# silverlight6/Ultrasound_Modeling

Measured on AMD Instinct MI355X. Metric: segmentation training images/sec at 256x256, higher is better.
Workload: dtype bf16

## Files before the change

### include/usseg.h

```cpp
#ifndef USSEG_H
#define USSEG_H

#include <stddef.h>
#include <stdint.h>

#ifdef __cplusplus
extern "C" {
#endif

typedef void* usseg_stream_t;

typedef enum UssegStatus {
  USSEG_OK = 0,
  USSEG_ERR_BAD_ARG = -1,
  USSEG_ERR_UNSUPPORTED = -2,
  USSEG_ERR_LAUNCH = -3
} UssegStatus;

typedef enum UssegAct { USSEG_ACT_NONE = 0, USSEG_ACT_LRELU = 1, USSEG_ACT_RELU = 2, USSEG_ACT_ELU = 3, USSEG_ACT_GELU = 4 } UssegAct;

enum {
  USSEG_OUT_F32 = 1,
  USSEG_ACCUMULATE = 2
};

typedef struct UssegConvDesc {
  int32_t B, H, W;
  int32_t Cin, Cout;
  int32_t ldx, ldy;
  int32_t ksize;
  int32_t dilation;
  int32_t act;
  float alpha;
  int32_t flags;
} UssegConvDesc;

const char* usseg_last_error(void);
int usseg_version(void);

int usseg_conv2d_fwd(const UssegConvDesc* d, const void* x, const void* wp_fwd, const float* bias,
                     const void* residual, int32_t ldr, void* y, usseg_stream_t stream);
int usseg_conv2d_fwd_affine(const UssegConvDesc* d, const void* x, const void* wp_fwd, const float* scale, const float* shift,
                            const void* residual, int32_t ldr, void* y, usseg_stream_t stream);
typedef struct UssegBnFoldJob {
  const float *gamma, *beta, *mean, *var;
  const float* bias;
  float *scale, *shift;
  int32_t C, Cp;
  float eps;
  int32_t reserved;
} UssegBnFoldJob;
int usseg_bn_fold_batched(const UssegBnFoldJob* jobs_dev, int32_t njobs, usseg_stream_t stream);
int usseg_conv2d_dgrad(const UssegConvDesc* d, const void* dy, const void* wp_dgrad, const void* residual,
                       int32_t ldr, void* dx, usseg_stream_t stream);
int usseg_conv2d_wgrad(const UssegConvDesc* d, const void* x, const void* dy, float* dw_scratch, float* ws,
                       int64_t ws_floats, usseg_stream_t stream);

int usseg_conv2d_dgrad_branches(const UssegConvDesc* d, int32_t nbranches, const int32_t* ksize, const int32_t* dilation,
                                const int32_t* ch_off, int32_t Cb, const void* dy, const void* wp_cat, const void* residual,
                                int32_t ldr, void* dx, usseg_stream_t stream);

typedef struct UssegWgradBlock {
  float* dst;
  int64_t sT, sI, sO;
  int32_t i_off, o_off, ni, no;
} UssegWgradBlock;
typedef struct UssegWgradDst {
  int32_t nblocks;
  int32_t reserved;
  UssegWgradBlock blk[4];
} UssegWgradDst;
int usseg_conv2d_wgrad_mapped(const UssegConvDesc* d, const void* x, const void* dy, const UssegWgradDst* dst, float* ws,
                              int64_t ws_floats, usseg_stream_t stream);
int usseg_tconv2d_wgrad_mapped(const UssegConvDesc* d, const void* x, const void* dy, const UssegWgradDst* dst, float* ws,
                               int64_t ws_floats, usseg_stream_t stream);

typedef struct UssegWgradJob {
  UssegConvDesc desc;
  const void* x;
  const void* dy;
  float* dw;
  const UssegWgradDst* dst;
} UssegWgradJob;
int usseg_conv2d_wgrad_multi(int32_t njobs, const UssegWgradJob* jobs, float* ws, int64_t ws_floats, usseg_stream_t stream);

int usseg_defer_begin(usseg_stream_t stream, float* reduce_ws, int64_t reduce_floats, float* wgrad_ws, int64_t wgrad_floats);
int usseg_defer_flush(usseg_stream_t stream);
int usseg_defer_end(usseg_stream_t stream);

typedef struct UssegConvJob {
  UssegConvDesc desc;
  const void* x;
  const void* wp;
  const float* bias;
  const void* residual;
  int32_t ldr;
  int32_t reserved;
  void* y;
  const float* scale;
} UssegConvJob;
int usseg_conv2d_fwd_multi(int32_t njobs, const UssegConvJob* jobs, usseg_stream_t stream);
int usseg_conv2d_dgrad_multi(int32_t njobs, const UssegConvJob* jobs, usseg_stream_t stream);

int usseg_tconv2d_fwd(const UssegConvDesc* d, const void* x, const void* wp_fwd, const float* bias, void* y,
                      usseg_stream_t stream);
int usseg_tconv2d_dgrad(const UssegConvDesc* d, const void* dy, const void* wp_dgrad, const void* residual,
                        int32_t ldr, void* dx, usseg_stream_t stream);
int usseg_tconv2d_wgrad(const UssegConvDesc* d, const void* x, const void* dy, float* dw_scratch,
                        usseg_stream_t stream);

int usseg_pack_weight(const float* src, int64_t sT, int64_t sN, int64_t sK, int32_t T, int32_t Nn, int32_t Kk,
                      void* dst, int32_t Kw, int32_t tap_stride, int32_t n_off, int32_t k_off,
                      usseg_stream_t stream);
typedef struct UssegPackJob {
  const float* src;
  void* dst;
  int64_t sT, sN, sK;
  int32_t T, Nn, Kk, Kw, tap_stride, n_off, k_off, reserved;
  const float* nscale;
} UssegPackJob;
int usseg_pack_weights_batched(const UssegPackJob* jobs_dev, int32_t njobs, usseg_stream_t stream);
int usseg_pack_weights_flat(const UssegPackJob* jobs_dev, const int32_t* tilemap_dev, int32_t nblocks, usseg_stream_t stream);
int usseg_unpack_wgrad(const float* scratch, int32_t Mrows, int32_t Ncols, int32_t T, int32_t Nn, int32_t Kk,
                       int32_t n_off, int32_t k_off, float* dst, int64_t sT, int64_t sN, int64_t sK,
                       float scale, int32_t accumulate, usseg_stream_t stream);
typedef struct UssegUnpackJob {
  const float* scratch;
  float* dst;
  int64_t sT, sN, sK;
  int32_t Mrows, Ncols, T, Nn, Kk, n_off, k_off, accumulate;
  float scale;
  int32_t reserved;
} UssegUnpackJob;
int usseg_unpack_wgrad_batched(const UssegUnpackJob* jobs_dev, int32_t njobs, int32_t max_elems, usseg_stream_t stream);

typedef struct UssegNormDesc {
  int64_t M;
  int32_t C, Cphys;
  int32_t ldx, ldy;
  int32_t G;
  int32_t mode;
  float eps;
  int32_t act;
  float alpha;
  int32_t lddx;
} UssegNormDesc;
int usseg_norm_act_fwd(const UssegNormDesc* d, const void* x, const float* gamma, const float* beta,
                       const float* mean, const float* var, const void* mask, int32_t ldm, void* y, usseg_stream_t stream);
int usseg_dropout_mask(void* mask, int64_t M, int32_t C, int32_t ld, uint64_t seed, float rate, usseg_stream_t stream);
int usseg_dropout_mask_step(void* mask, int64_t M, int32_t C, int32_t ld, uint64_t seed, const int32_t* step_dev, float rate,
                            usseg_stream_t stream);
int usseg_counter_add(int32_t* counter, int32_t inc, usseg_stream_t stream);
int usseg_norm_act_bwd(const UssegNormDesc* d, const void* x, const void* dy, const float* gamma, const float* beta,
                       const float* mean, const float* var, const void* mask, int32_t ldm, void* dx, float* dgamma,
                       float* dbeta, float* dbias, float* ws, usseg_stream_t stream);
int usseg_norm_act_bwd_res(const UssegNormDesc* d, const void* x, const void* dy, const float* gamma, const float* beta,
                           const void* dres, int32_t lddres, void* dx, float* dgamma, float* dbeta, float* dbias, float* ws,
                           usseg_stream_t stream);
int usseg_norm_act_fwd_gap(const UssegNormDesc* d, const void* x, const float* gamma, const float* beta, const float* mean,
                           const float* var, void* y, int32_t B, int32_t nb, float* gap_rows, usseg_stream_t stream);
int usseg_norm_act_bwd_sa(const UssegNormDesc* d, const void* x, const void* dout, const float* gamma, const float* beta,
                          const float* mean, const float* var, int32_t B, const float* sa_s, const float* sa_dg, float sa_mult,
                          void* dx, float* dgamma, float* dbeta, float* dbias, float* ws, usseg_stream_t stream);
int usseg_norm_act_bwd_pair(const UssegNormDesc* da, const void* xa, const void* dya, const float* gamma_a, const float* beta_a, void* dxa,
                            float* dgamma_a, float* dbeta_a, float* dbias_a, const UssegNormDesc* db, const void* xb, const void* doutb,
                            const float* gamma_b, const float* beta_b, int32_t B, const float* sa_s, const float* sa_dg, float sa_mult, void* dxb,
                            float* dgamma_b, float* dbeta_b, float* dbias_b, float* ws, usseg_stream_t stream);
int usseg_stem_fwd(int32_t B, int32_t H, int32_t W, const void* x, int32_t ldx, const void* w1, const float* b1, const void* w2, const float* b2,
                   const void* w3, const float* b3, const float* gamma, const float* beta, const float* mean, const float* var, float eps,
                   float alpha, void* y1, void* t1, void* c2, void* pooled, usseg_stream_t stream);
int usseg_stem_fwd_infer(int32_t B, int32_t H, int32_t W, const void* x, int32_t ldx, const void* w1, const float* b1, const void* w2,
                         const float* b2, const void* w3, const float* b3, const float* gamma, const float* beta, const float* mean,
                         const float* var, float eps, float alpha, void* pooled, usseg_stream_t stream);
int usseg_conv3_dgrad_actbwd(int32_t B, int32_t H, int32_t W, const void* dy, int32_t lddy, const void* wd, int32_t Co, const void* yact, int32_t ldy,
                             int32_t mode, const float* gamma, const float* beta, const float* var, float eps, float alpha, void* dx,
                             int32_t lddx, float* dgamma, float* dbeta, float* dbias, float* ws, usseg_stream_t stream);
typedef struct UssegCardinalDesc {
  int32_t B, H, W;
  int32_t Cin;
  int32_t P, cv11, cvkk;
  int32_t Up, Vp, Oc;
  int32_t ldx, ldu, ldv, ldsc;
  float eps, alpha;
} UssegCardinalDesc;
int32_t usseg_cardinal_supported(const UssegCardinalDesc* d);
int usseg_cardinal_fwd(const UssegCardinalDesc* d, const void* x, const void* w1, const float* b1, const float* g1, const float* be1,
                       const void* w2, const float* b2, const float* g2, const float* be2, const void* wsc, const float* bsc,
                       const float* gsc, const float* besc, void* u_raw, void* u, void* v_raw, void* y, float* gap_rows, void* sc_raw,
                       void* sc, usseg_stream_t stream);
int usseg_cardinal_fwd_infer(const UssegCardinalDesc* d, const void* x, const void* w1, const float* b1, const float* g1, const float* be1,
                             const void* w2, const float* b2, const float* g2, const float* be2, const void* wsc, const float* bsc,
                             const float* gsc, const float* besc, void* y, float* gap_rows, void* sc, usseg_stream_t stream);
int usseg_cardinal_bwd(const UssegCardinalDesc* d, const void* dout, int32_t ldo, const void* dsc, int32_t lddsc, const void* v_raw,
                       const void* u_raw, const void* sc_raw, const void* w2d, const float* g2, const float* be2, const float* g1,
                       const float* be1, const float* gsc, const float* besc, const float* sa_s, const float* sa_dg, float sa_mult, void* dv,
                       void* dcat, int32_t ldc, float* dg2, float* dbe2, float* db2, float* dg1, float* dbe1, float* db1, float* dgsc,
                       float* dbesc, float* dbsc, float* ws, usseg_stream_t stream);
int usseg_bn_act_pool_fwd(const void* x, int32_t B, int32_t H, int32_t W, int32_t C, int32_t Cphys, int32_t ldx, const float* gamma,
                          const float* beta, const float* mean, const float* var, float eps, int32_t act, float alpha, void* y,
                          int32_t ldy, usseg_stream_t stream);
int usseg_bn_act_pool_bwd(const void* x, const void* dy, int32_t B, int32_t H, int32_t W, int32_t C, int32_t Cphys, int32_t ldx,
                          int32_t lddy, const float* gamma, const float* beta, const float* mean, const float* var, float eps,
                          int32_t act, float alpha, void* dx, int32_t lddx, float* dgamma, float* dbeta, float* dbias, float* ws,
                          usseg_stream_t stream);
int64_t usseg_reduce_ws_floats(void);
int usseg_channel_stats(const void* x, int64_t M, int32_t C, int32_t ldx, float* sum, float* sumsq, float* ws,
                        usseg_stream_t stream);

int usseg_bn_finalize_stats(const float* sum, const float* sumsq, int64_t M, int32_t C, float momentum, float* mean, float* var,
                            float* moving_mean, float* moving_var, usseg_stream_t stream);
int usseg_bn_batch_stats(const void* x, int64_t M, int32_t C, int32_t ldx, float momentum, float* mean, float* var, float* moving_mean,
                         float* moving_var, float* ws, usseg_stream_t stream);
int usseg_bn_train_bwd_fix(const void* x, void* dx, int64_t M, int32_t C, int32_t Cphys, int32_t ldx, int32_t lddx, const float* gamma,
                           const float* mean, const float* var, float eps, const float* tg, const float* tb, usseg_stream_t stream);

int usseg_act_fwd(const void* x, int64_t M, int32_t C, int32_t ldx, int32_t ldy, int32_t act, float alpha, void* y,
                  usseg_stream_t stream);
int usseg_act_bwd(const void* x, const void* dy, int64_t M, int32_t C, int32_t ldx, int32_t lddy, int32_t lddx,
                  int32_t act, float alpha, void* dx, usseg_stream_t stream);
int usseg_act_bwd_colsum(const void* x, const void* dy, int64_t M, int32_t C, int32_t ldx, int32_t lddy, int32_t lddx, int32_t act,
                         float alpha, void* dx, float* db, float* ws, usseg_stream_t stream);

int usseg_avgpool2_fwd(const void* x, int32_t B, int32_t H, int32_t W, int32_t C, int32_t ldx, int32_t ldy, void* y,
                       usseg_stream_t stream);
int usseg_avgpool2_bwd(const void* dy, int32_t B, int32_t H, int32_t W, int32_t C, int32_t lddy, int32_t lddx,
                       const void* add, int32_t ldadd, void* dx, usseg_stream_t stream);
int usseg_avgpool2_bwd_colsum(const void* dy, int32_t B, int32_t H, int32_t W, int32_t C, int32_t lddy, int32_t lddx, const void* add,
                              int32_t ldadd, void* dx, float* db, float* ws, usseg_stream_t stream);

int usseg_copy_channels(const void* src, int64_t M, int32_t C, int32_t lds, void* dst, int32_t ldd, int32_t accumulate,
                        usseg_stream_t stream);
int usseg_cast_input(const void* src, int32_t src_is_f64, int64_t M, int32_t C, void* dst, int32_t Cphys,
                     usseg_stream_t stream);
int usseg_cast_bf16_to_f32(const void* src, int64_t M, int32_t C, int32_t lds, float* dst, usseg_stream_t stream);

typedef struct UssegSplitAttnDesc {
  int32_t B, HW;
  int32_t P, R, Cg, Hd;
  int32_t ldy, ldo;
  int32_t Cy_phys, Co_phys;
  float mult;
  int32_t norm_mode;
  float eps;
  int32_t act;
  float alpha;
  int32_t use_sigmoid;
} UssegSplitAttnDesc;
typedef struct UssegSplitAttnParams {
  const float *w1, *b1, *gamma, *beta, *mean, *var, *w2, *b2;
} UssegSplitAttnParams;
typedef struct UssegSplitAttnGrads {
  float *w1, *b1, *gamma, *beta, *w2, *b2;
} UssegSplitAttnGrads;
int usseg_splitattn_gap(const UssegSplitAttnDesc* d, const void* y, float* g, float* ws, usseg_stream_t stream);
int64_t usseg_splitattn_ws_floats(const UssegSplitAttnDesc* d);
int usseg_splitattn_mlp_fwd(const UssegSplitAttnDesc* d, const float* g, int32_t g_rows, int32_t g_stride,
                            const UssegSplitAttnParams* p, float* s, float* ws, usseg_stream_t stream);
int usseg_splitattn_apply_fwd(const UssegSplitAttnDesc* d, const void* y, const float* s, void* out,
                              usseg_stream_t stream);
int usseg_splitattn_apply_bwd_reduce(const UssegSplitAttnDesc* d, const void* y, const void* dout, int32_t lddo,
                                     float* ds, float* ws, usseg_stream_t stream);
int64_t usseg_splitattn_mlp_bwd_ws_floats(const UssegSplitAttnDesc* d);
int usseg_splitattn_mlp_bwd(const UssegSplitAttnDesc* d, const float* g, int32_t g_rows, int32_t g_stride,
                            const UssegSplitAttnParams* p, const float* s, const float* ws, const float* ds, float* dg,
                            const UssegSplitAttnGrads* grads, float* grad_ws, usseg_stream_t stream);
int usseg_splitattn_bwd_fused(const UssegSplitAttnDesc* d, const void* y, const void* dout, int32_t lddo, const float* g, int32_t g_rows,
                              int32_t g_stride, const UssegSplitAttnParams* p, const float* s, const float* ws, float* dg,
                              const UssegSplitAttnGrads* grads, float* reduce_ws, float* grad_ws, usseg_stream_t stream);
int usseg_splitattn_apply_bwd_dy(const UssegSplitAttnDesc* d, const void* dout, int32_t lddo, const float* s,
                                 const float* dg, void* dy, int32_t lddy, usseg_stream_t stream);

typedef struct UssegLossDesc {
  int64_t M;
  int32_t HW;
  int32_t C, ldl, lddl;
  int32_t loss_kind;
  float label_smoothing;
  float clip_eps;
  float inv_global_batch;
  int32_t quad_w;
} UssegLossDesc;
#define USSEG_ACC_FLOATS 2050
int usseg_softmax_loss_fwd_bwd(const UssegLossDesc* d, const float* logits, const float* y_true, const float* scale,
                               float* probs, float* loss, void* dlogits, usseg_stream_t stream);
int usseg_head_quad_softmax_loss(const void* x, int32_t B, int32_t h, int32_t w, int32_t Cin_phys, int32_t ldx, const void* wq, const float* bias, int32_t C,
                                 const float* y_true, float* probs, float* loss, void* dlogits, float label_smoothing, float clip_eps,
                                 float inv_global_batch, usseg_stream_t stream);
int usseg_accuracy(const float* probs, const float* y_true, int64_t M, int32_t C, float* acc, usseg_stream_t stream);
typedef struct UssegSegCountDesc {
  int32_t B, H, W, C;
  int32_t num_classes;
  int32_t round;
} UssegSegCountDesc;
#define USSEG_SEG_COUNTS 23
int usseg_seg_counts(const UssegSegCountDesc* d, const float* y_true, const float* y_pred, uint64_t* counts, usseg_stream_t stream);
int usseg_cascade_gate(const float* probs, int32_t C_mask, int64_t M, const void* x, int32_t ldx, void* x_gated, uint8_t* mask,
                       usseg_stream_t stream);
int usseg_cascade_maps(const float* probs, int32_t C, int64_t M, float* prob_map, float* bleed_prob, usseg_stream_t stream);
int usseg_loss_from_probs(const UssegLossDesc* d, const float* probs, const float* y_true, const float* scale, float* loss,
                          usseg_stream_t stream);
typedef struct UssegClassLoss {
  float w[8];
  float gamma;
  float factor;
} UssegClassLoss;
int usseg_softmax_loss_fwd_bwd_cl(const UssegLossDesc* d, const UssegClassLoss* cl, const float* logits, const float* y_true, float* probs,
                                  float* loss, void* dlogits, usseg_stream_t stream);
int usseg_head_quad_softmax_loss_cl(const void* x, int32_t B, int32_t h, int32_t w, int32_t Cin_phys, int32_t ldx, const void* wq, const float* bias,
                                    int32_t C, const float* y_true, float* probs, float* loss, void* dlogits, float label_smoothing, float clip_eps,
                                    float inv_global_batch, const UssegClassLoss* cl, usseg_stream_t stream);
int usseg_loss_from_probs_cl(const UssegLossDesc* d, const UssegClassLoss* cl, const float* probs, const float* y_true, float* loss,
                             int32_t as_map, usseg_stream_t stream);
typedef struct UssegOverlapLoss {
  float w[8];
  float alpha;
  float beta;
  float smooth;
  float power;
  float ov_weight;
  float ce_weight;
} UssegOverlapLoss;
#define USSEG_OVERLAP_ACC_FLOATS 8224
int usseg_overlap_loss_grid(int64_t M);
int usseg_overlap_loss_sums(const UssegLossDesc* d, const UssegOverlapLoss* ol, float ov_scale, const float* probs, const float* y_true,
                            float* acc, int64_t acc_floats, usseg_stream_t stream);
int usseg_overlap_loss_bwd(const UssegLossDesc* d, const UssegOverlapLoss* ol, const float* probs, const float* y_true, const float* acc,
                           int64_t acc_floats, void* dlogits, usseg_stream_t stream);
int64_t usseg_sdf_ws_bytes(int32_t B, int32_t H, int32_t W, int32_t C);
int usseg_sdf_labels(const float* y_true, int32_t B, int32_t H, int32_t W, int32_t C, float thr, float* phi, void* ws, int64_t ws_bytes,
                     usseg_stream_t stream);
int64_t usseg_surface_ws_bytes(int32_t N, int32_t H, int32_t W);
int usseg_surface_dist(const uint8_t* a, const uint8_t* b, int32_t N, int32_t H, int32_t W, int64_t* counters, double* sums, void* ws,
                       int64_t ws_bytes, usseg_stream_t stream);
int64_t usseg_surface_stats_ws_bytes(int32_t N, int32_t H, int32_t W);
int usseg_surface_stats(const uint8_t* a, const uint8_t* b, int32_t N, int32_t H, int32_t W, const double* quant, int32_t P, const int32_t* tol2,
                        int32_t T, int64_t* counters, double* sums, int32_t* sel, int64_t* within, void* ws, int64_t ws_bytes,
                        usseg_stream_t stream);
int64_t usseg_components_ws_bytes(int32_t N, int32_t H, int32_t W);
int usseg_label_components(const uint8_t* mask, int32_t N, int32_t H, int32_t W, int32_t connectivity, int32_t* labels, int32_t* count, void* ws,
                           int64_t ws_bytes, usseg_stream_t stream);
int usseg_component_stats(const int32_t* labels, const float* prob, int32_t N, int32_t H, int32_t W, int32_t cap, int64_t* stats,
                          usseg_stream_t stream);
int usseg_clean_mask(const uint8_t* mask, const float* prob, int32_t N, int32_t H, int32_t W, int32_t connectivity, int32_t min_area,
                     float min_peak, uint8_t* out, void* ws, int64_t ws_bytes, usseg_stream_t stream);
int usseg_component_overlap(const int32_t* labels_a, const int32_t* labels_b, int32_t N, int32_t H, int32_t W, int32_t cap_a, int32_t cap_b,
                            int32_t* hit_a, int32_t* hit_b, usseg_stream_t stream);
typedef struct UssegBoundaryLoss {
  float u[8];
} UssegBoundaryLoss;
int usseg_overlap_boundary_loss_sums(const UssegLossDesc* d, const UssegOverlapLoss* ol, float ov_scale, const float* probs, const float* y_true,
                                     const float* phi, const UssegBoundaryLoss* bl, const float* wb, float* acc, int64_t acc_floats,
                                     usseg_stream_t stream);
int usseg_overlap_boundary_loss_bwd(const UssegLossDesc* d, const UssegOverlapLoss* ol, const float* probs, const float* y_true, const float* phi,
                                    const UssegBoundaryLoss* bl, const float* acc, int64_t acc_floats, void* dlogits, usseg_stream_t stream);
#define USSEG_SORT_TILE 2048
#define USSEG_SORT_DIGIT_BITS 8
int64_t usseg_sort_ws_bytes(int32_t S, int64_t n);
int usseg_sort_pairs_u32(const uint32_t* keys_in, const uint32_t* vals_in, int32_t S, int64_t n, int32_t key_bits, uint32_t* keys_out,
                         uint32_t* vals_out, void* ws, int64_t ws_bytes, usseg_stream_t stream);
typedef struct UssegLovaszLoss {
  float w[8];
  float lv_weight;
  float ce_weight;
  float threshold;
  int32_t all_classes;
} UssegLovaszLoss;
int64_t usseg_lovasz_ws_bytes(int64_t M, int32_t C);
int usseg_lovasz_coeffs(const UssegLossDesc* d, UssegLovaszLoss ll, const float* probs, const float* y_true, float* g, int32_t* counts, void* ws,
                        int64_t ws_bytes, usseg_stream_t stream);
int usseg_lovasz_loss_sums(const UssegLossDesc* d, UssegLovaszLoss ll, float ov_scale, const float* probs, const float* y_true, const float* g,
                           const int32_t* counts, float* acc, int64_t acc_floats, usseg_stream_t stream);
int usseg_lovasz_loss_bwd(const UssegLossDesc* d, UssegLovaszLoss ll, const float* probs, const float* y_true, const float* g, const float* acc,
                          int64_t acc_floats, void* dlogits, usseg_stream_t stream);
int usseg_quad_bias_expand(const float* bias, int32_t C, int32_t Np, float* out , usseg_stream_t stream);
int usseg_quad_bias_fold(const float* d16 , int32_t C, float* dbias, usseg_stream_t stream);
int usseg_tconv_quad_unpack(const float* dq, int32_t Cin_phys, int32_t Cin, int32_t Cout, int32_t Np, int32_t ksize, float* grad,
                            usseg_stream_t stream);
int usseg_quad_head_fold(const float* dq, int32_t Cin_phys, int32_t Cin, int32_t Cout, int32_t Np, int32_t ksize, float* grad, const float* d16,
                         float* dbias, usseg_stream_t stream);
int usseg_space_to_depth2(const void* full, int32_t B, int32_t H, int32_t W, int32_t C, int32_t ld_full, void* quad, int32_t Np,
                          int32_t ld_quad, int32_t to_quad, usseg_stream_t stream);
int usseg_tconv_quad_fwd(const UssegConvDesc* d, int32_t ksize, int32_t Np, const void* x, const void* wq_f, const float* bias_q, void* y4,
                         usseg_stream_t stream);
int usseg_tconv_quad_dgrad(const UssegConvDesc* d, int32_t ksize, int32_t Np, const void* dy4, const void* wq_d, void* dx, usseg_stream_t stream);
int usseg_tconv_quad_wgrad(const UssegConvDesc* d, int32_t ksize, int32_t Np, const void* x, const void* dy4, float* dq, float* ws,
                           int64_t ws_floats, usseg_stream_t stream);

int usseg_loss_cat_scale(const float* y_true, int32_t B, int32_t HW, int32_t C, float* scale, usseg_stream_t stream);

int usseg_label2vec(const float* label, int64_t M, int32_t num_classes, float* out, usseg_stream_t stream);
typedef struct UssegAugSample {
  int32_t do_reduc, nclip;
  int32_t clip[2][4];
  int32_t do_shift, shift_r, shift_c, shift_dir;
  int32_t do_noise, do_flip;
  uint64_t seed;
} UssegAugSample;
typedef struct UssegAugDesc {
  int32_t B, H, W, C;
  int32_t Cphys;
  int32_t num_classes;
} UssegAugDesc;
int usseg_augment(const UssegAugDesc* d, const UssegAugSample* samples_dev, const void* x, int32_t x_is_f64, const float* y,
                  const float* noise, void* x_out_bf16, float* x_out_f32, float* y_out, float* y_vec, usseg_stream_t stream);

int usseg_reinject_hidden(void* hidden, int64_t numel, int32_t n, void* const* bufs, const int32_t* c0, const int32_t* ld,
                          int32_t backward, usseg_stream_t stream);

int usseg_patchify(const void* x, int32_t x_is_f64, int32_t B, int32_t H, int32_t W, int32_t C, int32_t patch, void* out, int32_t Cp,
                   usseg_stream_t stream);
int usseg_patch_merge(void* full, int32_t B, int32_t H, int32_t W, int32_t C, int32_t ldf, void* merged, int32_t ldm, int32_t backward,
                      usseg_stream_t stream);
int usseg_ln_wide_fwd(const void* x, int64_t M, int32_t C, int32_t ldx, const float* gamma, const float* beta, float eps, void* y,
                      int32_t ldy, usseg_stream_t stream);
int usseg_ln_wide_bwd(const void* x, const void* dy, int64_t M, int32_t C, int32_t ldx, int32_t lddy, const float* gamma, float eps,
                      void* dx, int32_t lddx, float* dgamma, float* dbeta, float* ws, int64_t ws_floats, usseg_stream_t stream);
int usseg_window_attn_fwd(const void* qkv, int32_t ldq, const float* table, int32_t B, int32_t H, int32_t W, int32_t C, int32_t heads,
                          int32_t ws, int32_t shift, void* out, int32_t ldo, usseg_stream_t stream);
int64_t usseg_window_attn_bwd_ws_floats(int32_t B, int32_t H, int32_t W, int32_t heads, int32_t ws);
int usseg_window_attn_bwd(const void* qkv, int32_t ldq, const void* dout, int32_t ldo, const float* table, int32_t B, int32_t H, int32_t W,
                          int32_t C, int32_t heads, int32_t ws, int32_t shift, void* dqkv, float* dtable, float* ws_rows,
                          usseg_stream_t stream);
int usseg_token_mean_fwd(const void* x, int32_t B, int32_t L, int32_t C, int32_t ld, float* out, usseg_stream_t stream);
int usseg_token_mean_bwd(const float* dy, int32_t B, int32_t L, int32_t C, int32_t ld, void* dx, usseg_stream_t stream);

int usseg_colsum(const void* dy, int64_t M, int32_t C, int32_t ld, float* db, float* ws, usseg_stream_t stream);

int usseg_sumsq(const float* g, int64_t n, float* out, usseg_stream_t stream);
int usseg_sum_f32(const float* x, int64_t n, float* out, usseg_stream_t stream);
int usseg_sumsq_advance(const float* g, int64_t n, float* out, int32_t* step, float* lr_t_dev, float lr, float beta1, float beta2,
                        usseg_stream_t stream);
int usseg_adam_clip_step(float* p, const float* g, float* m, float* v, int64_t n, const float* sumsq, float clip_norm,
                         const float* lr_t_dev, float beta1, float beta2, float eps, usseg_stream_t stream);
int usseg_adam_advance(int32_t* step, float* lr_t_dev, float lr, float beta1, float beta2, usseg_stream_t stream);
int usseg_fill_f32(float* p, int64_t n, float value, usseg_stream_t stream);
int usseg_scale_f32(float* p, int64_t n, const float* sumsq, float clip_norm, usseg_stream_t stream);

#define USSEG_SCHED_MAX_PIECES 16
typedef struct UssegLrSchedule {
  int32_t n;
  int32_t boundary[USSEG_SCHED_MAX_PIECES - 1];
  float lr[USSEG_SCHED_MAX_PIECES];
  float wd[USSEG_SCHED_MAX_PIECES];
} UssegLrSchedule;
int usseg_sched_advance(int32_t* step, const UssegLrSchedule* sched_dev, float* lr_t_dev, float* wd_t_dev, float beta1, float beta2,
                        usseg_stream_t stream);
int usseg_sumsq_sched_advance(const float* g, int64_t n, float* out, int32_t* step, const UssegLrSchedule* sched_dev, float* lr_t_dev,
                              float* wd_t_dev, float beta1, float beta2, usseg_stream_t stream);
int usseg_adamw_step(float* p, const float* g, float* m, float* v, int64_t n, const float* sumsq, float clip_norm, const float* lr_t_dev,
                     const float* wd_t_dev, const uint8_t* decay_mask, float beta1, float beta2, float eps, usseg_stream_t stream);

typedef struct UssegGemmDesc {
  int32_t M, N, K;
  int32_t ldx, ldw, ldy;
  int32_t nb1, nb2;
  int64_t xs1, xs2, ws1, ws2, ys1, ys2;
  int32_t flags;
} UssegGemmDesc;
int usseg_gemm_nt_batched(const UssegGemmDesc* d, const void* x, const void* w, void* y, usseg_stream_t stream);
int usseg_gemm_tn_batched(const UssegGemmDesc* d, const void* a, const void* b, float* out, usseg_stream_t stream);
int usseg_softmax_rows_fwd(const float* s, int64_t rows, int32_t n, float scale, float* p32, void* pbf, usseg_stream_t stream);
int usseg_softmax_rows_bwd(const float* p32, const float* dp, int64_t rows, int32_t n, float scale, void* ds_bf, usseg_stream_t stream);
int usseg_transpose_batched(const void* src, int32_t R, int32_t C, int32_t lds, int32_t nb1, int32_t nb2, int64_t ss1, int64_t ss2,
                            void* dst, usseg_stream_t stream);
int usseg_cast_f32_to_bf16_batched(const float* src, int32_t R, int32_t C, int32_t nb1, int32_t nb2, void* dst, int32_t ldd, int64_t ds1,
                                   int64_t ds2, usseg_stream_t stream);

typedef struct UssegFlashDesc {
  int32_t B, N, H, head_dim;
  int32_t ld_qkv, ld_o;
  float scale;
} UssegFlashDesc;
int usseg_flash_attn_fwd(const UssegFlashDesc* d, const void* q, const void* k, const void* v, void* o, float* o32, float* lse,
                         usseg_stream_t stream);
int usseg_flash_attn_bwd(const UssegFlashDesc* d, const void* q, const void* k, const void* v, const void* o, const float* o32,
                         const void* d_o, const float* lse, float* delta, void* dq, void* dk, void* dv, usseg_stream_t stream);

int usseg_prof_enable(int32_t kind_mask, int32_t capacity);
int usseg_prof_read(int32_t kind, double* total_ms, int64_t* launches);
int usseg_prof_disable(void);

#define USSEG_PREP_H 256
#define USSEG_PREP_W 80
int usseg_prep_cycle_stats(const double* frames, int32_t C, int32_t H0, int32_t W0, double* col_ws, double* stats, usseg_stream_t stream);
int usseg_prep_label(const double* brain, int32_t Hb, int32_t Wb, const double* blood, const double* normal, int32_t Hm, int32_t Wm,
                     int32_t objective, float* ws, float* label, uint8_t* gate, usseg_stream_t stream);
int usseg_prep_label_thick(const double* brain, int32_t Hb, int32_t Wb, const double* blood, int32_t Hm, int32_t Wm, int32_t order,
                           float* label, uint8_t* gate, usseg_stream_t stream);
int usseg_prep_assemble(const double* frames, const double* stats, int32_t C, int32_t H0, int32_t W0, const double* bmode, int32_t Hq,
                        int32_t Wq, int32_t F, const float* label, const uint8_t* gate, int32_t objective, double* out, usseg_stream_t stream);

int usseg_select_ranks_f64(const double* x, int32_t N, int64_t n, const int32_t* ranks, int32_t R, const int32_t* active, double* out,
                           usseg_stream_t stream);
#define USSEG_PREP_AUG_PARTIALS 64
typedef struct UssegPrepAugSample {
  int32_t do_flip, do_reduc, do_contrast, do_clip;
  int32_t clip[4];
  int32_t do_rotate, rot_slot;
  int32_t do_shift, shift_r, shift_c, shift_dir;
  int32_t do_noise, reserved;
  uint64_t seed;
  double rot[6];
} UssegPrepAugSample;
typedef struct UssegPrepAugDesc {
  int32_t N, H, W, C;
  int32_t n_rot;
  int32_t k_lo, k_hi;
  double g_lo, g_hi;
  double zH, zW;
} UssegPrepAugDesc;
int64_t usseg_prep_aug_ws_doubles(int32_t N, int32_t H, int32_t W, int32_t C, int32_t n_rot);
int usseg_prep_aug(const UssegPrepAugDesc* d, const UssegPrepAugSample* samples_dev, const int32_t* rot_list_dev, const double* x,
                   const double* noise, double* ws, int64_t ws_doubles, double* out, double* noise_out, usseg_stream_t stream);

int usseg_cone_index(const double* X, const double* Y, int32_t H, int32_t W, double xmin, double ymin, double ppu, int32_t Hp, int32_t Wp,
                     int32_t* index, usseg_stream_t stream);
int usseg_cone_range(const double* bmode, int32_t B, int32_t HW, double* range, int32_t* nonfinite, usseg_stream_t stream);
int usseg_cone_render(const int32_t* index, int32_t Hp, int32_t Wp, int32_t gap, const float* prob_map, const double* label, const float* bleed,
                      const double* bmode, int32_t B, int32_t H, int32_t W, const double* ranges, const double* bmode_range, const uint8_t* luts,
                      uint8_t* out, usseg_stream_t stream);

#define USSEG_ENSEMBLE_MAX 16
#define USSEG_CALIB_MAX_BINS 64
typedef struct UssegEnsembleDesc {
  int32_t B, H, W, C;
  int32_t K;
} UssegEnsembleDesc;
int usseg_ensemble_merge(const UssegEnsembleDesc* d, const float* const* members, uint32_t flip_w, float* mean_probs, float* entropy,
                         float* mutual_info, float* variance, usseg_stream_t stream);
int usseg_ensemble_image_scores(const UssegEnsembleDesc* d, const float* mean_probs, const float* entropy, const float* mutual_info,
                                float* scores, int32_t* counts, usseg_stream_t stream);
typedef struct UssegCalibDesc {
  int32_t B, H, W, C;
  int32_t bins;
  int32_t cls;
} UssegCalibDesc;
int usseg_calibration_bins(const UssegCalibDesc* d, const float* probs, const float* y_true, int64_t* counts, usseg_stream_t stream);

#ifdef __cplusplus
}
#endif
#endif
```

### ultrasound_modeling_amd/_lib.py

```python
from __future__ import annotations

import ctypes as C
import os

import torch
from . import knobs

_HERE = os.path.dirname(os.path.abspath(__file__))
LIB_PATH = knobs.get("USSEG_LIB") or os.path.join(_HERE, "libusseg_hip.so")

c_i32, c_i64, c_f32, c_vp = C.c_int32, C.c_int64, C.c_float, C.c_void_p


class UssegError(RuntimeError):
    pass


class ConvDesc(C.Structure):
    _fields_ = [("B", c_i32), ("H", c_i32), ("W", c_i32), ("Cin", c_i32), ("Cout", c_i32), ("ldx", c_i32),
                ("ldy", c_i32), ("ksize", c_i32), ("dilation", c_i32), ("act", c_i32), ("alpha", c_f32),
                ("flags", c_i32)]


class ConvJob(C.Structure):
    _fields_ = [("desc", ConvDesc), ("x", c_vp), ("wp", c_vp), ("bias", c_vp), ("residual", c_vp), ("ldr", c_i32),
                ("reserved", c_i32), ("y", c_vp), ("scale", c_vp)]


class WgradBlock(C.Structure):
    _fields_ = [("dst", c_vp), ("sT", c_i64), ("sI", c_i64), ("sO", c_i64), ("i_off", c_i32), ("o_off", c_i32), ("ni", c_i32), ("no", c_i32)]


class WgradDst(C.Structure):
    _fields_ = [("nblocks", c_i32), ("reserved", c_i32), ("blk", WgradBlock * 4)]


P_WgradDst = C.POINTER(WgradDst)


class WgradJob(C.Structure):
    _fields_ = [("desc", ConvDesc), ("x", c_vp), ("dy", c_vp), ("dw", c_vp), ("dst", P_WgradDst)]


class AugSample(C.Structure):
    _fields_ = [("do_reduc", c_i32), ("nclip", c_i32), ("clip", (c_i32 * 4) * 2), ("do_shift", c_i32), ("shift_r", c_i32),
                ("shift_c", c_i32), ("shift_dir", c_i32), ("do_noise", c_i32), ("do_flip", c_i32), ("seed", C.c_uint64)]


class AugDesc(C.Structure):
    _fields_ = [("B", c_i32), ("H", c_i32), ("W", c_i32), ("C", c_i32), ("Cphys", c_i32), ("num_classes", c_i32)]


class PrepAugSample(C.Structure):
    _fields_ = [("do_flip", c_i32), ("do_reduc", c_i32), ("do_contrast", c_i32), ("do_clip", c_i32), ("clip", c_i32 * 4), ("do_rotate", c_i32),
                ("rot_slot", c_i32), ("do_shift", c_i32), ("shift_r", c_i32), ("shift_c", c_i32), ("shift_dir", c_i32), ("do_noise", c_i32),
                ("reserved", c_i32), ("seed", C.c_uint64), ("rot", C.c_double * 6)]


class PrepAugDesc(C.Structure):
    _fields_ = [("N", c_i32), ("H", c_i32), ("W", c_i32), ("C", c_i32), ("n_rot", c_i32), ("k_lo", c_i32), ("k_hi", c_i32),
                ("g_lo", C.c_double), ("g_hi", C.c_double), ("zH", C.c_double), ("zW", C.c_double)]


class NormDesc(C.Structure):
    _fields_ = [("M", c_i64), ("C", c_i32), ("Cphys", c_i32), ("ldx", c_i32), ("ldy", c_i32), ("G", c_i32),
                ("mode", c_i32), ("eps", c_f32), ("act", c_i32), ("alpha", c_f32), ("lddx", c_i32)]


class CardinalDesc(C.Structure):
    _fields_ = [("B", c_i32), ("H", c_i32), ("W", c_i32), ("Cin", c_i32), ("P", c_i32), ("cv11", c_i32), ("cvkk", c_i32), ("Up", c_i32),
                ("Vp", c_i32), ("Oc", c_i32), ("ldx", c_i32), ("ldu", c_i32), ("ldv", c_i32), ("ldsc", c_i32), ("eps", c_f32), ("alpha", c_f32)]


class SplitAttnDesc(C.Structure):
    _fields_ = [("B", c_i32), ("HW", c_i32), ("P", c_i32), ("R", c_i32), ("Cg", c_i32), ("Hd", c_i32),
                ("ldy", c_i32), ("ldo", c_i32), ("Cy_phys", c_i32), ("Co_phys", c_i32), ("mult", c_f32),
                ("norm_mode", c_i32), ("eps", c_f32), ("act", c_i32), ("alpha", c_f32), ("use_sigmoid", c_i32)]


class SplitAttnParams(C.Structure):
    _fields_ = [(n, c_vp) for n in ("w1", "b1", "gamma", "beta", "mean", "var", "w2", "b2")]


class SplitAttnGrads(C.Structure):
    _fields_ = [(n, c_vp) for n in ("w1", "b1", "gamma", "beta", "w2", "b2")]


class GemmDesc(C.Structure):
    _fields_ = [("M", c_i32), ("N", c_i32), ("K", c_i32), ("ldx", c_i32), ("ldw", c_i32), ("ldy", c_i32), ("nb1", c_i32), ("nb2", c_i32),
                ("xs1", c_i64), ("xs2", c_i64), ("ws1", c_i64), ("ws2", c_i64), ("ys1", c_i64), ("ys2", c_i64), ("flags", c_i32)]


class ClassLoss(C.Structure):
    _fields_ = [("w", c_f32 * 8), ("gamma", c_f32), ("factor", c_f32)]


class OverlapLoss(C.Structure):
    _fields_ = [("w", c_f32 * 8), ("alpha", c_f32), ("beta", c_f32), ("smooth", c_f32), ("power", c_f32), ("ov_weight", c_f32),
                ("ce_weight", c_f32)]


class LovaszLoss(C.Structure):
    _fields_ = [("w", c_f32 * 8), ("lv_weight", c_f32), ("ce_weight", c_f32), ("threshold", c_f32), ("all_classes", c_i32)]


class BoundaryLoss(C.Structure):
    _fields_ = [("u", c_f32 * 8)]


class FlashDesc(C.Structure):
    _fields_ = [("B", c_i32), ("N", c_i32), ("H", c_i32), ("head_dim", c_i32), ("ld_qkv", c_i32), ("ld_o", c_i32), ("scale", c_f32)]


class LossDesc(C.Structure):
    _fields_ = [("M", c_i64), ("HW", c_i32), ("C", c_i32), ("ldl", c_i32), ("lddl", c_i32), ("loss_kind", c_i32),
                ("label_smoothing", c_f32), ("clip_eps", c_f32), ("inv_global_batch", c_f32), ("quad_w", c_i32)]


class SegCountDesc(C.Structure):
    _fields_ = [("B", c_i32), ("H", c_i32), ("W", c_i32), ("C", c_i32), ("num_classes", c_i32), ("round", c_i32)]


SEG_COUNTS = 23


class EnsembleDesc(C.Structure):
    _fields_ = [("B", c_i32), ("H", c_i32), ("W", c_i32), ("C", c_i32), ("K", c_i32)]


class CalibDesc(C.Structure):
    _fields_ = [("B", c_i32), ("H", c_i32), ("W", c_i32), ("C", c_i32), ("bins", c_i32), ("cls", c_i32)]


ENSEMBLE_MAX = 16
CALIB_MAX_BINS = 64

ACT_NONE, ACT_LRELU, ACT_RELU, ACT_ELU, ACT_GELU = 0, 1, 2, 3, 4
OUT_F32, ACCUMULATE = 1, 2

P = C.POINTER
_PROTOS = {
    "usseg_last_error": (C.c_char_p, []),
    "usseg_version": (C.c_int, []),
    "usseg_conv2d_fwd": (C.c_int, [P(ConvDesc), c_vp, c_vp, c_vp, c_vp, c_i32, c_vp, c_vp]),
    "usseg_conv2d_fwd_affine": (C.c_int, [P(ConvDesc), c_vp, c_vp, c_vp, c_vp, c_vp, c_i32, c_vp, c_vp]),
    "usseg_bn_fold_batched": (C.c_int, [c_vp, c_i32, c_vp]),
    "usseg_conv2d_dgrad": (C.c_int, [P(ConvDesc), c_vp, c_vp, c_vp, c_i32, c_vp, c_vp]),
    "usseg_conv2d_wgrad": (C.c_int, [P(ConvDesc), c_vp, c_vp, c_vp, c_vp, c_i64, c_vp]),
    "usseg_conv2d_wgrad_mapped": (C.c_int, [P(ConvDesc), c_vp, c_vp, P(WgradDst), c_vp, c_i64, c_vp]),
    "usseg_tconv2d_wgrad_mapped": (C.c_int, [P(ConvDesc), c_vp, c_vp, P(WgradDst), c_vp, c_i64, c_vp]),
    "usseg_conv2d_dgrad_branches": (C.c_int, [P(ConvDesc), c_i32, c_vp, c_vp, c_vp, c_i32, c_vp, c_vp, c_vp, c_i32, c_vp, c_vp]),
    "usseg_conv2d_wgrad_multi": (C.c_int, [c_i32, c_vp, c_vp, c_i64, c_vp]),
    "usseg_conv2d_fwd_multi": (C.c_int, [c_i32, c_vp, c_vp]),
    "usseg_conv2d_dgrad_multi": (C.c_int, [c_i32, c_vp, c_vp]),
    "usseg_tconv2d_fwd": (C.c_int, [P(ConvDesc), c_vp, c_vp, c_vp, c_vp, c_vp]),
    "usseg_tconv2d_dgrad": (C.c_int, [P(ConvDesc), c_vp, c_vp, c_vp, c_i32, c_vp, c_vp]),
    "usseg_tconv2d_wgrad": (C.c_int, [P(ConvDesc), c_vp, c_vp, c_vp, c_vp]),
    "usseg_pack_weight": (C.c_int, [c_vp, c_i64, c_i64, c_i64, c_i32, c_i32, c_i32, c_vp, c_i32, c_i32, c_i32, c_i32, c_vp]),
    "usseg_pack_weights_batched": (C.c_int, [c_vp, c_i32, c_vp]),
    "usseg_pack_weights_flat": (C.c_int, [c_vp, c_vp, c_i32, c_vp]),
    "usseg_unpack_wgrad": (C.c_int, [c_vp, c_i32, c_i32, c_i32, c_i32, c_i32, c_i32, c_i32, c_vp, c_i64, c_i64, c_i64,
                                     c_f32, c_i32, c_vp]),
    "usseg_unpack_wgrad_batched": (C.c_int, [c_vp, c_i32, c_i32, c_vp]),
    "usseg_norm_act_fwd": (C.c_int, [P(NormDesc), c_vp, c_vp, c_vp, c_vp, c_vp, c_vp, c_i32, c_vp, c_vp]),
    "usseg_dropout_mask": (C.c_int, [c_vp, c_i64, c_i32, c_i32, C.c_uint64, c_f32, c_vp]),
    "usseg_dropout_mask_step": (C.c_int, [c_vp, c_i64, c_i32, c_i32, C.c_uint64, c_vp, c_f32, c_vp]),
    "usseg_counter_add": (C.c_int, [c_vp, c_i32, c_vp]),
    "usseg_norm_act_bwd": (C.c_int, [P(NormDesc), c_vp, c_vp, c_vp, c_vp, c_vp, c_vp, c_vp, c_i32, c_vp, c_vp, c_vp, c_vp, c_vp, c_vp]),
    "usseg_bn_act_pool_fwd": (C.c_int, [c_vp, c_i32, c_i32, c_i32, c_i32, c_i32, c_i32, c_vp, c_vp, c_vp, c_vp, c_f32, c_i32, c_f32, c_vp, c_i32, c_vp]),
    "usseg_bn_act_pool_bwd": (C.c_int, [c_vp, c_vp, c_i32, c_i32, c_i32, c_i32, c_i32, c_i32, c_i32, c_vp, c_vp, c_vp, c_vp, c_f32, c_i32, c_f32,
                                        c_vp, c_i32, c_vp, c_vp, c_vp, c_vp, c_vp]),
    "usseg_reduce_ws_floats": (c_i64, []),
    "usseg_channel_stats": (C.c_int, [c_vp, c_i64, c_i32, c_i32, c_vp, c_vp, c_vp, c_vp]),
    "usseg_bn_finalize_stats": (C.c_int, [c_vp, c_vp, c_i64, c_i32, c_f32, c_vp, c_vp, c_vp, c_vp, c_vp]),
    "usseg_bn_batch_stats": (C.c_int, [c_vp, c_i64, c_i32, c_i32, c_f32, c_vp, c_vp, c_vp, c_vp, c_vp, c_vp]),
    "usseg_bn_train_bwd_fix": (C.c_int, [c_vp, c_vp, c_i64, c_i32, c_i32, c_i32, c_i32, c_vp, c_vp, c_vp, c_f32, c_vp, c_vp, c_vp]),
    "usseg_act_fwd": (C.c_int, [c_vp, c_i64, c_i32, c_i32, c_i32, c_i32, c_f32, c_vp, c_vp]),
    "usseg_act_bwd": (C.c_int, [c_vp, c_vp, c_i64, c_i32, c_i32, c_i32, c_i32, c_i32, c_f32, c_vp, c_vp]),
    "usseg_act_bwd_colsum": (C.c_int, [c_vp, c_vp, c_i64, c_i32, c_i32, c_i32, c_i32, c_i32, c_f32, c_vp, c_vp, c_vp, c_vp]),
    "usseg_avgpool2_fwd": (C.c_int, [c_vp, c_i32, c_i32, c_i32, c_i32, c_i32, c_i32, c_vp, c_vp]),
    "usseg_avgpool2_bwd": (C.c_int, [c_vp, c_i32, c_i32, c_i32, c_i32, c_i32, c_i32, c_vp, c_i32, c_vp, c_vp]),
    "usseg_avgpool2_bwd_colsum": (C.c_int, [c_vp, c_i32, c_i32, c_i32, c_i32, c_i32, c_i32, c_vp, c_i32, c_vp, c_vp, c_vp, c_vp]),
    "usseg_copy_channels": (C.c_int, [c_vp, c_i64, c_i32, c_i32, c_vp, c_i32, c_i32, c_vp]),
    "usseg_cast_input": (C.c_int, [c_vp, c_i32, c_i64, c_i32, c_vp, c_i32, c_vp]),
    "usseg_cast_bf16_to_f32": (C.c_int, [c_vp, c_i64, c_i32, c_i32, c_vp, c_vp]),
    "usseg_splitattn_gap": (C.c_int, [P(SplitAttnDesc), c_vp, c_vp, c_vp, c_vp]),
    "usseg_splitattn_ws_floats": (c_i64, [P(SplitAttnDesc)]),
    "usseg_splitattn_mlp_fwd": (C.c_int, [P(SplitAttnDesc), c_vp, c_i32, c_i32, P(SplitAttnParams), c_vp, c_vp, c_vp]),
    "usseg_norm_act_fwd_gap": (C.c_int, [P(NormDesc), c_vp, c_vp, c_vp, c_vp, c_vp, c_vp, c_i32, c_i32, c_vp, c_vp]),
    "usseg_stem_fwd": (C.c_int, [c_i32, c_i32, c_i32, c_vp, c_i32, c_vp, c_vp, c_vp, c_vp, c_vp, c_vp, c_vp, c_vp, c_vp, c_vp, c_f32, c_f32,
                                 c_vp, c_vp, c_vp, c_vp, c_vp]),
    "usseg_stem_fwd_infer": (C.c_int, [c_i32, c_i32, c_i32, c_vp, c_i32, c_vp, c_vp, c_vp, c_vp, c_vp, c_vp, c_vp, c_vp, c_vp, c_vp, c_f32, c_f32,
                                       c_vp, c_vp]),
    "usseg_conv3_dgrad_actbwd": (C.c_int, [c_i32, c_i32, c_i32, c_vp, c_i32, c_vp, c_i32, c_vp, c_i32, c_i32, c_vp, c_vp, c_vp, c_f32, c_f32, c_vp, c_i32,
                                           c_vp, c_vp, c_vp, c_vp, c_vp]),
    "usseg_cardinal_supported": (c_i32, [P(CardinalDesc)]),
    "usseg_cardinal_fwd": (C.c_int, [P(CardinalDesc)] + [c_vp] * 21),
    "usseg_cardinal_fwd_infer": (C.c_int, [P(CardinalDesc)] + [c_vp] * 17),
    "usseg_cardinal_bwd": (C.c_int, [P(CardinalDesc), c_vp, c_i32, c_vp, c_i32] + [c_vp] * 12 + [c_f32, c_vp, c_vp, c_i32] + [c_vp] * 11),
    "usseg_accuracy": (C.c_int, [c_vp, c_vp, c_i64, c_i32, c_vp, c_vp]),
    "usseg_seg_counts": (C.c_int, [P(SegCountDesc), c_vp, c_vp, c_vp, c_vp]),
    "usseg_cascade_gate": (C.c_int, [c_vp, c_i32, c_i64, c_vp, c_i32, c_vp, c_vp, c_vp]),
    "usseg_cascade_maps": (C.c_int, [c_vp, c_i32, c_i64, c_vp, c_vp, c_vp]),
    "usseg_norm_act_bwd_res": (C.c_int, [P(NormDesc), c_vp, c_vp, c_vp, c_vp, c_vp, c_i32, c_vp, c_vp, c_vp, c_vp, c_vp, c_vp]),
    "usseg_norm_act_bwd_sa": (C.c_int, [P(NormDesc), c_vp, c_vp, c_vp, c_vp, c_vp, c_vp, c_i32, c_vp, c_vp, c_f32, c_vp, c_vp, c_vp, c_vp, c_vp, c_vp]),
    "usseg_norm_act_bwd_pair": (C.c_int, [P(NormDesc)] + [c_vp] * 8 + [P(NormDesc)] + [c_vp] * 4 + [c_i32, c_vp, c_vp, c_f32] + [c_vp] * 6),
    "usseg_splitattn_apply_fwd": (C.c_int, [P(SplitAttnDesc), c_vp, c_vp, c_vp, c_vp]),
    "usseg_splitattn_apply_bwd_reduce": (C.c_int, [P(SplitAttnDesc), c_vp, c_vp, c_i32, c_vp, c_vp, c_vp]),
    "usseg_splitattn_mlp_bwd_ws_floats": (c_i64, [P(SplitAttnDesc)]),
    "usseg_splitattn_bwd_fused": (C.c_int, [P(SplitAttnDesc), c_vp, c_vp, c_i32, c_vp, c_i32, c_i32, P(SplitAttnParams), c_vp, c_vp, c_vp,
                                            P(SplitAttnGrads), c_vp, c_vp, c_vp]),
    "usseg_splitattn_mlp_bwd": (C.c_int, [P(SplitAttnDesc), c_vp, c_i32, c_i32, P(SplitAttnParams), c_vp, c_vp, c_vp, c_vp,
                                          P(SplitAttnGrads), c_vp, c_vp]),
    "usseg_splitattn_apply_bwd_dy": (C.c_int, [P(SplitAttnDesc), c_vp, c_i32, c_vp, c_vp, c_vp, c_i32, c_vp]),
    "usseg_softmax_loss_fwd_bwd": (C.c_int, [P(LossDesc), c_vp, c_vp, c_vp, c_vp, c_vp, c_vp, c_vp]),
    "usseg_head_quad_softmax_loss": (C.c_int, [c_vp, c_i32, c_i32, c_i32, c_i32, c_i32, c_vp, c_vp, c_i32, c_vp, c_vp, c_vp, c_vp, c_f32, c_f32, c_f32, c_vp]),
    "usseg_loss_from_probs": (C.c_int, [P(LossDesc), c_vp, c_vp, c_vp, c_vp, c_vp]),
    "usseg_softmax_loss_fwd_bwd_cl": (C.c_int, [P(LossDesc), P(ClassLoss), c_vp, c_vp, c_vp, c_vp, c_vp, c_vp]),
    "usseg_head_quad_softmax_loss_cl": (C.c_int, [c_vp, c_i32, c_i32, c_i32, c_i32, c_i32, c_vp, c_vp, c_i32, c_vp, c_vp, c_vp, c_vp, c_f32, c_f32, c_f32,
                                                  P(ClassLoss), c_vp]),
    "usseg_loss_from_probs_cl": (C.c_int, [P(LossDesc), P(ClassLoss), c_vp, c_vp, c_vp, c_i32, c_vp]),
    "usseg_overlap_loss_grid": (C.c_int, [c_i64]),
    "usseg_overlap_loss_sums": (C.c_int, [P(LossDesc), P(OverlapLoss), c_f32, c_vp, c_vp, c_vp, c_i64, c_vp]),
    "usseg_overlap_loss_bwd": (C.c_int, [P(LossDesc), P(OverlapLoss), c_vp, c_vp, c_vp, c_i64, c_vp, c_vp]),
    "usseg_sdf_ws_bytes": (c_i64, [c_i32, c_i32, c_i32, c_i32]),
    "usseg_sdf_labels": (C.c_int, [c_vp, c_i32, c_i32, c_i32, c_i32, c_f32, c_vp, c_vp, c_i64, c_vp]),
    "usseg_surface_ws_bytes": (c_i64, [c_i32, c_i32, c_i32]),
    "usseg_surface_dist": (C.c_int, [c_vp, c_vp, c_i32, c_i32, c_i32, c_vp, c_vp, c_vp, c_i64, c_vp]),
    "usseg_surface_stats_ws_bytes": (c_i64, [c_i32, c_i32, c_i32]),
    "usseg_surface_stats": (C.c_int, [c_vp, c_vp, c_i32, c_i32, c_i32, c_vp, c_i32, c_vp, c_i32, c_vp, c_vp, c_vp, c_vp, c_vp, c_i64, c_vp]),
    "usseg_components_ws_bytes": (c_i64, [c_i32, c_i32, c_i32]),
    "usseg_label_components": (C.c_int, [c_vp, c_i32, c_i32, c_i32, c_i32, c_vp, c_vp, c_vp, c_i64, c_vp]),
    "usseg_component_stats": (C.c_int, [c_vp, c_vp, c_i32, c_i32, c_i32, c_i32, c_vp, c_vp]),
    "usseg_clean_mask": (C.c_int, [c_vp, c_vp, c_i32, c_i32, c_i32, c_i32, c_i32, c_f32, c_vp, c_vp, c_i64, c_vp]),
    "usseg_component_overlap": (C.c_int, [c_vp, c_vp, c_i32, c_i32, c_i32, c_i32, c_i32, c_vp, c_vp, c_vp]),
    "usseg_overlap_boundary_loss_sums": (C.c_int, [P(LossDesc), P(OverlapLoss), c_f32, c_vp, c_vp, c_vp, P(BoundaryLoss), c_vp, c_vp, c_i64, c_vp]),
    "usseg_overlap_boundary_loss_bwd": (C.c_int, [P(LossDesc), P(OverlapLoss), c_vp, c_vp, c_vp, P(BoundaryLoss), c_vp, c_i64, c_vp, c_vp]),
    "usseg_sort_ws_bytes": (c_i64, [c_i32, c_i64]),
    "usseg_sort_pairs_u32": (C.c_int, [c_vp, c_vp, c_i32, c_i64, c_i32, c_vp, c_vp, c_vp, c_i64, c_vp]),
    "usseg_lovasz_ws_bytes": (c_i64, [c_i64, c_i32]),
    "usseg_lovasz_coeffs": (C.c_int, [P(LossDesc), LovaszLoss, c_vp, c_vp, c_vp, c_vp, c_vp, c_i64, c_vp]),
    "usseg_lovasz_loss_sums": (C.c_int, [P(LossDesc), LovaszLoss, c_f32, c_vp, c_vp, c_vp, c_vp, c_vp, c_i64, c_vp]),
    "usseg_lovasz_loss_bwd": (C.c_int, [P(LossDesc), LovaszLoss, c_vp, c_vp, c_vp, c_vp, c_i64, c_vp, c_vp]),
    "usseg_quad_bias_expand": (C.c_int, [c_vp, c_i32, c_i32, c_vp, c_vp]),
    "usseg_space_to_depth2": (C.c_int, [c_vp, c_i32, c_i32, c_i32, c_i32, c_i32, c_vp, c_i32, c_i32, c_i32, c_vp]),
    "usseg_tconv_quad_fwd": (C.c_int, [P(ConvDesc), c_i32, c_i32, c_vp, c_vp, c_vp, c_vp, c_vp]),
    "usseg_tconv_quad_dgrad": (C.c_int, [P(ConvDesc), c_i32, c_i32, c_vp, c_vp, c_vp, c_vp]),
    "usseg_tconv_quad_wgrad": (C.c_int, [P(ConvDesc), c_i32, c_i32, c_vp, c_vp, c_vp, c_vp, c_i64, c_vp]),
    "usseg_quad_bias_fold": (C.c_int, [c_vp, c_i32, c_vp, c_vp]),
    "usseg_tconv_quad_unpack": (C.c_int, [c_vp, c_i32, c_i32, c_i32, c_i32, c_i32, c_vp, c_vp]),
    "usseg_quad_head_fold": (C.c_int, [c_vp, c_i32, c_i32, c_i32, c_i32, c_i32, c_vp, c_vp, c_vp, c_vp]),
    "usseg_label2vec": (C.c_int, [c_vp, c_i64, c_i32, c_vp, c_vp]),
    "usseg_augment": (C.c_int, [P(AugDesc), c_vp, c_vp, c_i32, c_vp, c_vp, c_vp, c_vp, c_vp, c_vp, c_vp]),
    "usseg_loss_cat_scale": (C.c_int, [c_vp, c_i32, c_i32, c_i32, c_vp, c_vp]),
    "usseg_patchify": (C.c_int, [c_vp, c_i32, c_i32, c_i32, c_i32, c_i32, c_i32, c_vp, c_i32, c_vp]),
    "usseg_patch_merge": (C.c_int, [c_vp, c_i32, c_i32, c_i32, c_i32, c_i32, c_vp, c_i32, c_i32, c_vp]),
    "usseg_ln_wide_fwd": (C.c_int, [c_vp, c_i64, c_i32, c_i32, c_vp, c_vp, c_f32, c_vp, c_i32, c_vp]),
    "usseg_ln_wide_bwd": (C.c_int, [c_vp, c_vp, c_i64, c_i32, c_i32, c_i32, c_vp, c_f32, c_vp, c_i32, c_vp, c_vp, c_vp, c_i64, c_vp]),
    "usseg_window_attn_fwd": (C.c_int, [c_vp, c_i32, c_vp, c_i32, c_i32, c_i32, c_i32, c_i32, c_i32, c_i32, c_vp, c_i32, c_vp]),
    "usseg_window_attn_bwd_ws_floats": (c_i64, [c_i32, c_i32, c_i32, c_i32, c_i32]),
    "usseg_window_attn_bwd": (C.c_int, [c_vp, c_i32, c_vp, c_i32, c_vp, c_i32, c_i32, c_i32, c_i32, c_i32, c_i32, c_i32, c_vp, c_vp, c_vp, c_vp]),
    "usseg_token_mean_fwd": (C.c_int, [c_vp, c_i32, c_i32, c_i32, c_i32, c_vp, c_vp]),
    "usseg_token_mean_bwd": (C.c_int, [c_vp, c_i32, c_i32, c_i32, c_i32, c_vp, c_vp]),
    "usseg_colsum": (C.c_int, [c_vp, c_i64, c_i32, c_i32, c_vp, c_vp, c_vp]),
    "usseg_sumsq": (C.c_int, [c_vp, c_i64, c_vp, c_vp]),
    "usseg_sum_f32": (C.c_int, [c_vp, c_i64, c_vp, c_vp]),
    "usseg_sumsq_advance": (C.c_int, [c_vp, c_i64, c_vp, c_vp, c_vp, c_f32, c_f32, c_f32, c_vp]),
    "usseg_reinject_hidden": (C.c_int, [c_vp, c_i64, c_i32, c_vp, c_vp, c_vp, c_i32, c_vp]),
    "usseg_adam_clip_step": (C.c_int, [c_vp, c_vp, c_vp, c_vp, c_i64, c_vp, c_f32, c_vp, c_f32, c_f32, c_f32, c_vp]),
    "usseg_adam_advance": (C.c_int, [c_vp, c_vp, c_f32, c_f32, c_f32, c_vp]),
    "usseg_fill_f32": (C.c_int, [c_vp, c_i64, c_f32, c_vp]),
    "usseg_scale_f32": (C.c_int, [c_vp, c_i64, c_vp, c_f32, c_vp]),
    "usseg_sched_advance": (C.c_int, [c_vp, c_vp, c_vp, c_vp, c_f32, c_f32, c_vp]),
    "usseg_sumsq_sched_advance": (C.c_int, [c_vp, c_i64, c_vp, c_vp, c_vp, c_vp, c_vp, c_f32, c_f32, c_vp]),
    "usseg_adamw_step": (C.c_int, [c_vp, c_vp, c_vp, c_vp, c_i64, c_vp, c_f32, c_vp, c_vp, c_vp, c_f32, c_f32, c_f32, c_vp]),
    "usseg_gemm_nt_batched": (C.c_int, [P(GemmDesc), c_vp, c_vp, c_vp, c_vp]),
    "usseg_gemm_tn_batched": (C.c_int, [P(GemmDesc), c_vp, c_vp, c_vp, c_vp]),
    "usseg_flash_attn_fwd": (C.c_int, [P(FlashDesc), c_vp, c_vp, c_vp, c_vp, c_vp, c_vp, c_vp]),
    "usseg_flash_attn_bwd": (C.c_int, [P(FlashDesc), c_vp, c_vp, c_vp, c_vp, c_vp, c_vp, c_vp, c_vp, c_vp, c_vp, c_vp, c_vp]),
    "usseg_softmax_rows_fwd": (C.c_int, [c_vp, c_i64, c_i32, c_f32, c_vp, c_vp, c_vp]),
    "usseg_softmax_rows_bwd": (C.c_int, [c_vp, c_vp, c_i64, c_i32, c_f32, c_vp, c_vp]),
    "usseg_transpose_batched": (C.c_int, [c_vp, c_i32, c_i32, c_i32, c_i32, c_i32, c_i64, c_i64, c_vp, c_vp]),
    "usseg_cast_f32_to_bf16_batched": (C.c_int, [c_vp, c_i32, c_i32, c_i32, c_i32, c_vp, c_i32, c_i64, c_i64, c_vp]),
    "usseg_defer_begin": (C.c_int, [c_vp, c_vp, c_i64, c_vp, c_i64]),
    "usseg_defer_flush": (C.c_int, [c_vp]),
    "usseg_defer_end": (C.c_int, [c_vp]),
    "usseg_prof_enable": (C.c_int, [c_i32, c_i32]),
    "usseg_prof_read": (C.c_int, [c_i32, P(C.c_double), P(c_i64)]),
    "usseg_prof_disable": (C.c_int, []),
    "usseg_prep_cycle_stats": (C.c_int, [c_vp, c_i32, c_i32, c_i32, c_vp, c_vp, c_vp]),
    "usseg_prep_label": (C.c_int, [c_vp, c_i32, c_i32, c_vp, c_vp, c_i32, c_i32, c_i32, c_vp, c_vp, c_vp, c_vp]),
    "usseg_prep_label_thick": (C.c_int, [c_vp, c_i32, c_i32, c_vp, c_i32, c_i32, c_i32, c_vp, c_vp, c_vp]),
    "usseg_prep_assemble": (C.c_int, [c_vp, c_vp, c_i32, c_i32, c_i32, c_vp, c_i32, c_i32, c_i32, c_vp, c_vp, c_i32, c_vp, c_vp]),
    "usseg_select_ranks_f64": (C.c_int, [c_vp, c_i32, c_i64, P(c_i32), c_i32, c_vp, c_vp, c_vp]),
    "usseg_prep_aug_ws_doubles": (c_i64, [c_i32, c_i32, c_i32, c_i32, c_i32]),
    "usseg_prep_aug": (C.c_int, [P(PrepAugDesc), c_vp, c_vp, c_vp, c_vp, c_vp, c_i64, c_vp, c_vp, c_vp]),
    "usseg_cone_index": (C.c_int, [c_vp, c_vp, c_i32, c_i32, C.c_double, C.c_double, C.c_double, c_i32, c_i32, c_vp, c_vp]),
    "usseg_cone_range": (C.c_int, [c_vp, c_i32, c_i32, c_vp, c_vp, c_vp]),
    "usseg_cone_render": (C.c_int, [c_vp, c_i32, c_i32, c_i32, c_vp, c_vp, c_vp, c_vp, c_i32, c_i32, c_i32, P(C.c_double), c_vp, c_vp, c_vp,
                                    c_vp]),
    "usseg_ensemble_merge": (C.c_int, [P(EnsembleDesc), P(c_vp), C.c_uint32, c_vp, c_vp, c_vp, c_vp, c_vp]),
    "usseg_ensemble_image_scores": (C.c_int, [P(EnsembleDesc), c_vp, c_vp, c_vp, c_vp, c_vp, c_vp]),
    "usseg_calibration_bins": (C.c_int, [P(CalibDesc), c_vp, c_vp, c_vp, c_vp]),
}
EXPORTED_SYMBOLS = tuple(_PROTOS)

_lib = None


def load() -> C.CDLL:
    global _lib
    if _lib is not None:
        return _lib
    if not os.path.exists(LIB_PATH):
        raise UssegError(f"{LIB_PATH} not found: build the HIP extension first (python -c 'import __graft_entry__ as g; "
                         f"g.build()'). There is no CPU fallback.")
    lib = C.CDLL(LIB_PATH)
    for name, (res, args) in _PROTOS.items():
        fn = getattr(lib, name)
        fn.restype = res
        fn.argtypes = args
    _lib = lib
    return lib


def check(rc: int, what: str = "") -> None:
    if rc != 0:
        msg = load().usseg_last_error().decode("utf-8", "replace")
        raise UssegError(f"{what}: usseg error {rc}: {msg}")
```

### ultrasound_modeling_amd/csrc/knobs.h

```cpp
#pragma once
#include <stdint.h>
#include <stdlib.h>

#define USSEG_KNOBS(X)                                                                                                                  \
                                                                                                                      \
  X(K_BIG,                "USSEG_BIG",                INT,     1,     ONCE,     "0: conv_big and the streaming conv take no launch")        \
  X(K_BIG_PX,             "USSEG_BIG_PX",             INT,     0,     ONCE,     "conv_big: force the pixel tile (128 / 256; 0: planner)")   \
  X(K_BIG_NT,             "USSEG_BIG_NT",             INT,     0,     ONCE,     "conv_big: force the channel tile (1 / 2 / 4 x 16; 0: planner)") \
  X(K_BIG_MIN_WG,         "USSEG_BIG_MIN_WG",         INT,     128,   ONCE,     "conv_big: smallest launch it takes, in workgroups")        \
  X(K_BIG_WG_TILE,        "USSEG_BIG_WG_TILE",        INT,     512,   ONCE,     "conv_big: narrow the channel tile below this many workgroups") \
  X(K_BIG_MIN_CIN,        "USSEG_BIG_MIN_CIN",        INT,     33,    ONCE,     "conv_big: fewest input channels of a pass it takes")       \
  X(K_BIG_STAGES,         "USSEG_BIG_STAGES",         INT,     0,     ONCE,     "conv_big LDS stages: 0 by launch size, 1 / 2 forced")      \
  X(K_BIG_W8,             "USSEG_BIG_W8",             INT,     1,     PER_CALL, "256-pixel tile on eight waves: 0 never, 1 planner, 2 forced") \
  X(K_BIG_W8_MIN,         "USSEG_BIG_W8_MIN",         INT,     128,   ONCE,     "fewest workgroups left for the eight-wave tile")           \
  X(K_STREAM,             "USSEG_STREAM",             INT,     1,     ONCE,     "0: the streaming conv takes no launch")                    \
  X(K_STREAM_PX,          "USSEG_STREAM_PX",          INT,     0,     ONCE,     "streaming conv: force the pixel tile (128 / 256; 0: planner)") \
  X(K_STREAM_MIN_STEPS,   "USSEG_STREAM_MIN_STEPS",   INT,     1,     PER_CALL, "streaming conv: fewest K steps per workgroup it takes")    \
  X(K_STREAM_WGX,         "USSEG_STREAM_WGX",         INT,     0,     PER_CALL, "streaming conv: force grid.x (>= 8, rounded down to a multiple of 8)") \
  X(K_STREAM_OCC,         "USSEG_STREAM_OCC",         INT,     0,     ONCE,     "streaming conv: cap on workgroups per CU (0: by LDS)")     \
  X(K_STREAM_RES,         "USSEG_STREAM_RES",         INT,     1,     ONCE,     "0: passes with a residual do not stream")                  \
  X(K_STREAM_MULTI,       "USSEG_STREAM_MULTI",       INT,     1,     ONCE,     "0: multi-job launches do not stream")                      \
  X(K_STREAM_MERGE,       "USSEG_STREAM_MERGE",       INT,     1,     PER_CALL, "streaming jobs of one plan in one launch (0: a launch per job)") \
                                                                                                     \
  X(K_NO_HALO,            "USSEG_NO_HALO",            PRESENT, 0,     ONCE,     "the halo-tile conv and weight-gradient kernels take no launch") \
  X(K_NO_PERSIST,         "USSEG_NO_PERSIST",         PRESENT, 0,     ONCE,     "conv_halo: never the persistent variant")                  \
  X(K_PERSIST_OCC,        "USSEG_PERSIST_OCC",        INT,     0,     ONCE,     "persistent conv_halo: workgroups per CU (0: by LDS)")      \
                                                                                                                    \
  X(K_IGEMM_WG_MIN,       "USSEG_IGEMM_WG_MIN",       INT,     256,   ONCE,     "igemm: narrow the channel tile below this many workgroups") \
  X(K_IGEMM_KC,           "USSEG_IGEMM_KC",           INT,     0,     ONCE,     "register-staged igemm: force the K step (4 / 8 chunks; 0: by K length)") \
  X(K_IGEMM_DMA,          "USSEG_IGEMM_DMA",          INT,     1,     ONCE,     "0: never the LDS-DMA igemm")                               \
  X(K_IGEMM_DMA_MIN,      "USSEG_IGEMM_DMA_MIN",      INT,     4,     ONCE,     "LDS-DMA igemm: fewest K chunks it takes")                  \
  X(K_IGEMM_DMA_BATCHED,  "USSEG_IGEMM_DMA_BATCHED",  INT,     1,     ONCE,     "0: batched GEMMs stay on the register-staged igemm")       \
  X(K_IGEMM_XCD,          "USSEG_IGEMM_XCD",          INT,     1,     ONCE,     "XCD-aware item order: 0 off, 1 activation-heavy launches, 2 all") \
  X(K_IGEMM_PERSIST,      "USSEG_IGEMM_PERSIST",      INT,     1,     ONCE,     "0: never the persistent LDS-DMA igemm")                    \
  X(K_IGEMM_STAGES8,      "USSEG_IGEMM_STAGES8",      INT,     4,     ONCE,     "ring depth of sparse long-K 128-channel launches (2: off, 3, 4)") \
  X(K_IGEMM_STAGES8_WG,   "USSEG_IGEMM_STAGES8_WG",   INT,     256,   ONCE,     "largest launch, in workgroups, that gets the deeper ring") \
                                                                                                         \
  X(K_WGRAD_DMA,          "USSEG_WGRAD_DMA",          INT,     1,     ONCE,     "0: never the LDS-DMA per-tap weight gradient / batched TN GEMM") \
  X(K_WGRAD_TM,           "USSEG_WGRAD_TM",           INT,     0,     ONCE,     "per-tap wgrad: force the tile (1: 64x64, 2: 128x128; 0: planner)") \
  X(K_WGD_TARGET,         "USSEG_WGD_TARGET",         INT,     512,   ONCE,     "per-tap wgrad: workgroups the split-K aims for")           \
  X(K_WGD_CAP,            "USSEG_WGD_CAP",            INT,     4,     ONCE,     "per-tap wgrad: slab traffic cap, in multiples of the operand bytes") \
  X(K_WG_QUANT,           "USSEG_WG_QUANT",           INT,     1,     ONCE,     "0: no wave-quantisation search of the split count (both wgrad kernels)") \
  X(K_WGRAD_DEBUG,        "USSEG_WGRAD_DEBUG",        PRESENT, 0,     ONCE,     "print every weight-gradient plan to stderr")               \
  X(K_WGRAD_POW2,         "USSEG_WGRAD_POW2",         INT,     1,     ONCE,     "0: no shift decode of power-of-two grids")                 \
  X(K_WGRAD_XCD,          "USSEG_WGRAD_XCD",          INT,     1,     ONCE,     "0: no XCD-aware item order in the per-tap wgrad")          \
  X(K_WG_TARGET,          "USSEG_WG_TARGET",          INT,     256,   ONCE,     "halo wgrad: workgroups the split-K aims for")              \
  X(K_SLAB_CAP,           "USSEG_SLAB_CAP",           INT,     2,     ONCE,     "halo wgrad: slab traffic cap, in multiples of the operand bytes") \
  X(K_WGHALO_XCD,         "USSEG_WGHALO_XCD",         INT,     1,     ONCE,     "0: no XCD-aware item order in the halo wgrad")             \
  X(K_WGRAD_PF,           "USSEG_WGRAD_PF",           INT,     1,     ONCE,     "0: halo wgrad without the register prefetch")              \
  X(K_WGRAD_8W,           "USSEG_WGRAD_8W",           INT,     1,     ONCE,     "0: the 64x64 halo wgrad tile on four waves, not eight")    \
  X(K_TCONV_HALO,         "USSEG_TCONV_HALO",         INT,     0,     PER_CALL, "1: transposed-conv wgrad as four parity-class halo jobs")  \
                                                                                                                      \
  X(K_CARD_BWD_G,         "USSEG_CARD_BWD_G",         INT,     0,     ONCE,     "fused cardinal backward: force the workgroup pairs (0: one resident wave)") \
  X(K_LN_TILE,            "USSEG_LN_TILE",            INT,     1,     ONCE,     "0: never the tile LayerNorm backward")                     \
  X(K_LN_PAIR,            "USSEG_LN_PAIR",            INT,     1,     ONCE,     "0: never the paired LayerNorm backward launch")            \
  X(K_LN_TILE_MIN,        "USSEG_LN_TILE_MIN",        INT,     32768, ONCE,     "fewest pixels for the tile / paired LayerNorm backward")   \
                                                                                     \
  X(K_FLASH_TILE,         "USSEG_FLASH_TILE",         INT,     -1,    ONCE,     "fused attention tiling 0 / 1 / 2 (-1: by problem size)")   \
  X(K_WINATTN_MFMA,       "USSEG_WINATTN_MFMA",       INT,     1,     ONCE,     "0: window attention without the MFMA kernels")             \
  X(K_LOSS_PPT,           "USSEG_LOSS_PPT",           INT,     4,     ONCE,     "softmax + loss kernel: pixels per thread")

enum Knob {
#define X(id, name, kind, def, life, doc) id,
  USSEG_KNOBS(X)
#undef X
};
enum { KNOB_INT, KNOB_PRESENT, KNOB_ONCE, KNOB_PER_CALL };
struct KnobDef { const char* name; int kind; int64_t def; int life; };
constexpr KnobDef kKnobs[] = {
#define X(id, name, kind, def, life, doc) {name, KNOB_##kind, def, KNOB_##life},
  USSEG_KNOBS(X)
#undef X
};

template <Knob K>
__attribute__((visibility("hidden"))) inline int64_t knob() {
  auto read = [] {
    const char* v = getenv(kKnobs[K].name);
    return kKnobs[K].kind == KNOB_PRESENT ? (int64_t)(v != nullptr) : (v ? (int64_t)atoll(v) : kKnobs[K].def);
  };
  if constexpr (kKnobs[K].life == KNOB_PER_CALL) return read();
  else {
    static const int64_t v = read();
    return v;
  }
}
```

### ultrasound_modeling_amd/csrc/wgrad.hip

```cpp
#include "common.h"

struct WgradParams {
  const bf16_t* a;
  const bf16_t* b;
  float* out;
  int32_t B, Hg, Wg;
  int64_t M;
  int32_t Ha, Wa, lda, asy, asx;
  int32_t Hb, Wb, ldb, bsy, bsx;
  int32_t Ma, Nb;
  int32_t mtiles, ntiles;
  int64_t chunk;
  int16_t ady[16], adx[16], bdy[16], bdx[16];
  int32_t nb2;
  int64_t as1, as2, bs1, bs2, os1, os2;
  WgMap map;
  float* ws;
  int32_t ntaps;
  int32_t xcd_remap;
  int32_t lw, lh;
};

__global__ __launch_bounds__(256) void wgrad_kernel(const WgradParams p) {
  constexpr int BK = 32, TS = 72;
  __shared__ __attribute__((aligned(16))) bf16_t lds[2][2][BK * TS];

  const int tid = threadIdx.x, lane = tid & 63, wv = tid >> 6;
  const int t = p.nb2 > 0 ? 0 : (int)blockIdx.z;
  const int bz1 = p.nb2 > 0 ? (int)blockIdx.z / p.nb2 : 0, bz2 = p.nb2 > 0 ? (int)blockIdx.z - bz1 * p.nb2 : 0;
  const bf16_t* const abase = p.a + bz1 * p.as1 + bz2 * p.as2;
  const bf16_t* const bbase = p.b + bz1 * p.bs1 + bz2 * p.bs2;
  const int mt = blockIdx.y / p.ntiles, nt = blockIdx.y - mt * p.ntiles;
  const int m0 = mt * 64, n0 = nt * 64;
  const int64_t k_begin = (int64_t)blockIdx.x * p.chunk;
  int64_t k_end = k_begin + p.chunk;
  if (k_end > p.M) k_end = p.M;
  if (k_begin >= k_end) return;
  const int ady = p.ady[t], adx = p.adx[t], bdy = p.bdy[t], bdx = p.bdx[t];
  const int HWg = p.Hg * p.Wg;

  const int pr = tid >> 3, cc = tid & 7;
  const bool a_ok = (m0 + cc * 8) < p.Ma, b_ok = (n0 + cc * 8) < p.Nb;
  uint4 ra, rb;
  auto load_step = [&](int64_t kbase) {
    int64_t m = kbase + pr;
    ra = make_uint4(0, 0, 0, 0);
    rb = ra;
    if (m < k_end) {
      int mm = (int)m;
      int b = mm / HWg;
      int rem = mm - b * HWg;
      int gy = rem / p.Wg, gx = rem - gy * p.Wg;
      int ay = gy * p.asy + ady, ax = gx * p.asx + adx;
      int by = gy * p.bsy + bdy, bx = gx * p.bsx + bdx;
      bool in_a = (unsigned)ay < (unsigned)p.Ha && (unsigned)ax < (unsigned)p.Wa;
      bool in_b = (unsigned)by < (unsigned)p.Hb && (unsigned)bx < (unsigned)p.Wb;
      if (in_a && in_b) {
        if (a_ok) ra = *reinterpret_cast<const uint4*>(abase + ((int64_t)(b * p.Ha + ay) * p.Wa + ax) * p.lda + m0 + cc * 8);
        if (b_ok) rb = *reinterpret_cast<const uint4*>(bbase + ((int64_t)(b * p.Hb + by) * p.Wb + bx) * p.ldb + n0 + cc * 8);
      }
    }
  };
  auto store_step = [&](int buf) {
    *reinterpret_cast<uint4*>(&lds[buf][0][pr * TS + cc * 8]) = ra;
    *reinterpret_cast<uint4*>(&lds[buf][1][pr * TS + cc * 8]) = rb;
  };

  const int wm = wv >> 1, wn = wv & 1;
  f32x4_t acc[2][2];
#pragma unroll
  for (int i = 0; i < 2; ++i)
#pragma unroll
    for (int j = 0; j < 2; ++j) acc[i][j] = (f32x4_t){0.f, 0.f, 0.f, 0.f};

  const int g = lane >> 4, li = lane & 15, tq = li >> 2, tp = li & 3;
  auto frag = [&](const bf16_t* tile, int col0) -> bf16x8_t {
    const bf16_t* a0 = tile + (8 * g + tq) * TS + col0 + 4 * tp;
    s16x4_t lo = __builtin_amdgcn_ds_read_tr16_b64_v4i16((s16x4_t __attribute__((address_space(3)))*)(a0));
    s16x4_t hi = __builtin_amdgcn_ds_read_tr16_b64_v4i16((s16x4_t __attribute__((address_space(3)))*)(a0 + 4 * TS));
    typedef __attribute__((ext_vector_type(8))) short s16x8_t;
    s16x8_t v = {lo[0], lo[1], lo[2], lo[3], hi[0], hi[1], hi[2], hi[3]};
    return __builtin_bit_cast(bf16x8_t, v);
  };

  load_step(k_begin);
  store_step(0);
  __syncthreads();
  int it = 0;
  for (int64_t kb = k_begin; kb < k_end; kb += BK, ++it) {
    const int cur = it & 1;
    const bool more = (kb + BK) < k_end;
    if (more) load_step(kb + BK);
    bf16x8_t af[2], bfr[2];
#pragma unroll
    for (int i = 0; i < 2; ++i) {
      af[i] = frag(&lds[cur][0][0], wm * 32 + i * 16);
      bfr[i] = frag(&lds[cur][1][0], wn * 32 + i * 16);
    }
#pragma unroll
    for (int i = 0; i < 2; ++i)
#pragma unroll
      for (int j = 0; j < 2; ++j) acc[i][j] = __builtin_amdgcn_mfma_f32_16x16x32_bf16(af[i], bfr[j], acc[i][j], 0, 0, 0);
    if (more) store_step(cur ^ 1);
    __syncthreads();
  }

  float* out = p.out + (int64_t)t * p.Ma * p.Nb + bz1 * p.os1 + bz2 * p.os2;
  float* slab = p.ws ? p.ws + ((int64_t)blockIdx.x * p.ntaps + t) * p.Ma * p.Nb : nullptr;
#pragma unroll
  for (int i = 0; i < 2; ++i)
#pragma unroll
    for (int j = 0; j < 2; ++j) {
      int n = n0 + wn * 32 + j * 16 + li;
      if (n >= p.Nb) continue;
#pragma unroll
      for (int r = 0; r < 4; ++r) {
        int m = m0 + wm * 32 + i * 16 + g * 4 + r;
        if (m >= p.Ma) continue;
        if (slab) slab[(int64_t)m * p.Nb + n] = acc[i][j][r];
        else {
          float* q = wg_map_dst(p.map, out, (int64_t)m * p.Nb + n, t, m, n);
          if (q) atomicAdd(q, acc[i][j][r]);
        }
      }
    }
}

typedef __attribute__((address_space(3))) void* wg_lds_ptr_t;
#define WGRAD_OOB 0x80000000u
typedef int wg_i32x4_t __attribute__((ext_vector_type(4)));
__device__ __forceinline__ wg_i32x4_t wg_rsrc(const void* base) {
  const uint64_t a = (uint64_t)base;
  return (wg_i32x4_t){(int)(uint32_t)a, (int)((uint32_t)(a >> 32) & 0xffffu), 0x7fffffff, 0x00020000};
}
__device__ __forceinline__ void wg_dma16(const wg_i32x4_t rsrc, char* lds_dst, uint32_t voff) {
  const uint32_t la = (uint32_t)(uintptr_t)(__attribute__((address_space(3))) char*)lds_dst;
  asm volatile("s_mov_b32 m0, %0\n\ts_nop 0\n\tbuffer_load_dwordx4 %1, %2, 0 offen lds" ::"s"(la), "v"(voff), "s"(rsrc) : "memory");
}

template <int TM, int NSTAGE>
__global__ __launch_bounds__(256, 2) void wgrad_dma_kernel(const WgradParams p, const float rcp_hw, const float rcp_w) {
#if defined(__HIP_DEVICE_COMPILE__)
  constexpr int BT = 64 * TM;
  constexpr int ROWB = BT * 2;
  constexpr int OPB = 64 * ROWB;
  constexpr int STAGE = 2 * OPB;
  constexpr int RPI = 1024 / ROWB;
  constexpr int IT = 64 / RPI / 4;
  constexpr int NI = 2 * IT;
  constexpr int D = NSTAGE - 1;
  constexpr int MT = 2 * TM;
  extern __shared__ __attribute__((aligned(1024))) char lds_raw[];

  const int tid = threadIdx.x, lane = tid & 63, wv = __builtin_amdgcn_readfirstlane(tid >> 6);
  int bx = blockIdx.x, by = blockIdx.y, bz = blockIdx.z;
  if (p.xcd_remap) {
    const int gx = gridDim.x, gy = gridDim.y, gz = gridDim.z, total = gx * gy * gz;
    const int L = bx + gx * (by + gy * bz);
    const int c = L & 7, q = total >> 3, r = total & 7;
    const int item = c * q + (c < r ? c : r) + (L >> 3);
    const int u = __builtin_amdgcn_readfirstlane(fdiv(item, fdiv_rcp(gz)));
    bz = item - u * gz;
    bx = __builtin_amdgcn_readfirstlane(fdiv(u, fdiv_rcp(gy)));
    by = u - bx * gy;
  }
  const int t = p.nb2 > 0 ? 0 : bz;
  const int bz1 = p.nb2 > 0 ? bz / p.nb2 : 0, bz2 = p.nb2 > 0 ? bz - bz1 * p.nb2 : 0;
  const int mt = by / p.ntiles, nt = by - mt * p.ntiles;
  const int m0 = mt * BT, n0 = nt * BT;
  const int64_t k_begin = (int64_t)bx * p.chunk;
  int64_t k_end = k_begin + p.chunk;
  if (k_end > p.M) k_end = p.M;
  if (k_begin >= k_end) return;
  const int nks = (int)((k_end - k_begin + 63) >> 6);
  const int ady = p.ady[t], adx = p.adx[t], bdy = p.bdy[t], bdx = p.bdx[t];
  const int HWg = p.Hg * p.Wg;

  const wg_i32x4_t ra = wg_rsrc(p.a + bz1 * p.as1 + bz2 * p.as2);
  const wg_i32x4_t rb = wg_rsrc(p.b + bz1 * p.bs1 + bz2 * p.bs2);

  const int lrow = TM == 1 ? (lane >> 3) : (lane >> 4);
  const int slot = TM == 1 ? (lane & 7) : (lane & 15);
  const int fkey = TM == 1 ? ((lane >> 4) & 3) : ((4 * (wv & 1) + (lane >> 4)) & 7);
  const int ch = (((slot >> 1) ^ fkey) << 4) + ((slot & 1) << 3);
  const bool a_cok = (m0 + ch) < p.Ma, b_cok = (n0 + ch) < p.Nb;
  const int a_c = m0 + ch, b_c = n0 + ch;

  const bool linear = p.asy == 1 && p.asx == 1 && p.bsy == 1 && p.bsx == 1 && ady == 0 && adx == 0 && bdy == 0 && bdx == 0 &&
                      p.Ha == p.Hg && p.Wa == p.Wg && p.Hb == p.Hg && p.Wb == p.Wg;
  int kpos = 0;
  int lin_m[IT];
  uint32_t lin_a[IT], lin_b[IT];
#pragma unroll
  for (int it = 0; it < IT; ++it) {
    lin_m[it] = (int)k_begin + RPI * (wv + 4 * it) + lrow;
    lin_a[it] = ((uint32_t)lin_m[it] * (uint32_t)p.lda + (uint32_t)a_c) * 2u;
    lin_b[it] = ((uint32_t)lin_m[it] * (uint32_t)p.ldb + (uint32_t)b_c) * 2u;
  }
  const uint32_t lin_sa = 128u * (uint32_t)p.lda, lin_sb = 128u * (uint32_t)p.ldb;
  const int k_end_i = (int)k_end;
  auto issue = [&](int stage) {
    char* const sa = lds_raw + stage * STAGE;
    char* const sb = sa + OPB;
    if (linear) {
#pragma unroll
      for (int it = 0; it < IT; ++it) {
        const int j = wv + 4 * it;
        const bool pv = lin_m[it] < k_end_i;
        wg_dma16(ra, sa + j * 1024, (pv & a_cok) ? lin_a[it] : WGRAD_OOB);
        wg_dma16(rb, sb + j * 1024, (pv & b_cok) ? lin_b[it] : WGRAD_OOB);
        lin_m[it] += 64; lin_a[it] += lin_sa; lin_b[it] += lin_sb;
      }
      kpos += 64;
      return;
    }
#pragma unroll
    for (int it = 0; it < IT; ++it) {
      const int j = wv + 4 * it;
      const int64_t m = k_begin + kpos + RPI * j + lrow;
      const bool pv = m < k_end;
      const int mm = pv ? (int)m : 0;
      int b, gy, gx;
      if (p.lw >= 0) {
        gx = mm & (p.Wg - 1);
        gy = (mm >> p.lw) & (p.Hg - 1);
        b = mm >> (p.lw + p.lh);
      } else {
        b = (int)((float)mm * rcp_hw);
        int rem = mm - __mul24(b, HWg);
        if (rem < 0) { --b; rem += HWg; }
        if (rem >= HWg) { ++b; rem -= HWg; }
        gy = (int)((float)rem * rcp_w);
        gx = rem - __mul24(gy, p.Wg);
        if (gx < 0) { --gy; gx += p.Wg; }
        if (gx >= p.Wg) { ++gy; gx -= p.Wg; }
      }
      const int ay = __mul24(gy, p.asy) + ady, ax = __mul24(gx, p.asx) + adx;
      const int by = __mul24(gy, p.bsy) + bdy, bx = __mul24(gx, p.bsx) + bdx;
      const bool in_a = ((unsigned)ay < (unsigned)p.Ha) & ((unsigned)ax < (unsigned)p.Wa);
      const bool in_b = ((unsigned)by < (unsigned)p.Hb) & ((unsigned)bx < (unsigned)p.Wb);
      const bool oka = pv & in_a & in_b & a_cok;
      const bool okb = pv & in_b & b_cok;
      const uint32_t offa = (__umul24((uint32_t)(__mul24(__mul24(b, p.Ha) + ay, p.Wa) + ax), (uint32_t)p.lda) + (uint32_t)a_c) * 2u;
      const uint32_t offb = (__umul24((uint32_t)(__mul24(__mul24(b, p.Hb) + by, p.Wb) + bx), (uint32_t)p.ldb) + (uint32_t)b_c) * 2u;
      wg_dma16(ra, sa + j * 1024, oka ? offa : WGRAD_OOB);
      wg_dma16(rb, sb + j * 1024, okb ? offb : WGRAD_OOB);
    }
    kpos += 64;
  };

  const int wm = wv >> 1, wn = wv & 1;
  f32x4_t acc[MT][MT];
#pragma unroll
  for (int i = 0; i < MT; ++i)
#pragma unroll
    for (int j = 0; j < MT; ++j) acc[i][j] = (f32x4_t){0.f, 0.f, 0.f, 0.f};

  const int g = lane >> 4, li = lane & 15, tq = li >> 2, tp = li & 3;
  typedef __attribute__((ext_vector_type(8))) short s16x8_t;
  auto tr8 = [&](const char* a0, const char* a1) -> bf16x8_t {
    s16x4_t lo = __builtin_amdgcn_ds_read_tr16_b64_v4i16((s16x4_t __attribute__((address_space(3)))*)(a0));
    s16x4_t hi = __builtin_amdgcn_ds_read_tr16_b64_v4i16((s16x4_t __attribute__((address_space(3)))*)(a1));
    s16x8_t v = {lo[0], lo[1], lo[2], lo[3], hi[0], hi[1], hi[2], hi[3]};
    return __builtin_bit_cast(bf16x8_t, v);
  };
  auto frag_off = [&](int r, int blk) -> int {
    const int f = TM == 1 ? ((r >> 1) & 3) : (r & 7);
    return r * ROWB + ((blk ^ f) << 5) + (tp << 3);
  };

#pragma unroll
  for (int s = 0; s < D; ++s)
    if (s < nks) issue(s);
  for (int ks = 0; ks < nks; ++ks) {
    static_assert(D <= 3, "the wait ladder below covers up to three stages in flight");
    if (D >= 3 && ks + 2 < nks) asm volatile("s_waitcnt vmcnt(%0) lgkmcnt(0)\n\ts_barrier" ::"n"(2 * NI) : "memory");
    else if (D >= 2 && ks + 1 < nks) asm volatile("s_waitcnt vmcnt(%0) lgkmcnt(0)\n\ts_barrier" ::"n"(NI) : "memory");
    else asm volatile("s_waitcnt vmcnt(0) lgkmcnt(0)\n\ts_barrier" ::: "memory");
    if (ks + D < nks) issue((ks + D) % NSTAGE);
    const char* const LA = lds_raw + (ks % NSTAGE) * STAGE;
    const char* const LB = LA + OPB;
#pragma unroll
    for (int kk = 0; kk < 2; ++kk) {
      const int r0 = 32 * kk + 4 * g + tq, r1 = r0 + 16;
      bf16x8_t af[MT], bfr[MT];
#pragma unroll
      for (int i = 0; i < MT; ++i) {
        af[i] = tr8(LA + frag_off(r0, wm * MT + i), LA + frag_off(r1, wm * MT + i));
        bfr[i] = tr8(LB + frag_off(r0, wn * MT + i), LB + frag_off(r1, wn * MT + i));
      }
#pragma unroll
      for (int i = 0; i < MT; ++i)
#pragma unroll
        for (int j = 0; j < MT; ++j) acc[i][j] = __builtin_amdgcn_mfma_f32_16x16x32_bf16(bfr[j], af[i], acc[i][j], 0, 0, 0);
    }
  }

  float* out = p.out + (int64_t)t * p.Ma * p.Nb + bz1 * p.os1 + bz2 * p.os2;
  float* slab = p.ws ? p.ws + ((int64_t)bx * p.ntaps + t) * p.Ma * p.Nb : nullptr;
  const bool vec_ok = (p.Nb & 3) == 0;
#pragma unroll
  for (int i = 0; i < MT; ++i)
#pragma unroll
    for (int j = 0; j < MT; ++j) {
      const int m = m0 + (wm * MT + i) * 16 + li;
      const int n = n0 + (wn * MT + j) * 16 + g * 4;
      if (m >= p.Ma || n >= p.Nb) continue;
      if (slab && vec_ok && n + 3 < p.Nb) {
        *reinterpret_cast<float4*>(slab + (int64_t)m * p.Nb + n) = make_float4(acc[i][j][0], acc[i][j][1], acc[i][j][2], acc[i][j][3]);
      } else {
#pragma unroll
        for (int r = 0; r < 4; ++r) {
          if (n + r >= p.Nb) continue;
          if (slab) slab[(int64_t)m * p.Nb + n + r] = acc[i][j][r];
          else {
            float* q = wg_map_dst(p.map, out, (int64_t)m * p.Nb + n + r, t, m, n + r);
            if (q) atomicAdd(q, acc[i][j][r]);
          }
        }
      }
    }
#endif
}

template <int TM, int NSTAGE>
static void wgrad_dma_launch_t(const WgradParams& p, dim3 grid, hipStream_t s) {
  const size_t dyn = (size_t)NSTAGE * 2 * 64 * 64 * TM * 2;
  if (usseg_lds_opt_in((const void*)wgrad_dma_kernel<TM, NSTAGE>, 128 * 1024)) return;
  hipLaunchKernelGGL((wgrad_dma_kernel<TM, NSTAGE>), grid, dim3(256), dyn, s, p, 1.0f / (float)(p.Hg * p.Wg), 1.0f / (float)p.Wg);
}

static int launch_wgrad(WgradParams& p, int ntaps, float* ws, int64_t ws_floats, hipStream_t s) {
  const int dma_env = knob<K_WGRAD_DMA>();
  const bool dma = dma_env && p.nb2 <= 0 && p.M < (1 << 24) && (int64_t)p.Hg * p.Wg < (1 << 23) && (int64_t)p.B * p.Ha * p.Wa < (1 << 24) && (int64_t)p.B * p.Hb * p.Wb < (1 << 24) &&
                   (int64_t)p.B * p.Ha * p.Wa * p.lda * 2 < 0x7fff0000ll &&
                   (int64_t)p.B * p.Hb * p.Wb * p.ldb * 2 < 0x7fff0000ll && p.lda % 8 == 0 && p.ldb % 8 == 0;
  const int tm_env = knob<K_WGRAD_TM>();
  int tm = 1;
  if (dma && p.Ma > 64 && p.Nb > 64) tm = 2;
  if (dma && tm_env) tm = tm_env;
  const int bt = 64 * tm;
  p.mtiles = (p.Ma + bt - 1) / bt;
  p.ntiles = (p.Nb + bt - 1) / bt;
  p.ntaps = ntaps;
  int64_t tiles = (int64_t)p.mtiles * p.ntiles * ntaps;
  const int wg_target = knob<K_WGD_TARGET>();
  const int slab_cap = knob<K_WGD_CAP>();
  int64_t want = (wg_target + tiles - 1) / tiles;
  int64_t max_splits = cdiv64(p.M, 256);
  if (want > max_splits) want = max_splits;
  if (want < 1) want = 1;
  const int64_t slab = (int64_t)ntaps * p.Ma * p.Nb;
  p.ws = nullptr;
  int64_t cap_splits = 1;
  if (ws) ws = usseg_defer_wgrad_ws(s, ws, ws_floats, &ws_floats);
  if (ws && want > 1) {
    const int64_t in_bytes = p.M * (p.Ma + p.Nb) * 2;
    int64_t cap = slab_cap * in_bytes / (slab * 4);
    if (cap < 4) cap = 4;
    if (cap > ws_floats / slab) cap = ws_floats / slab;
    if (want > cap) want = cap;
    cap_splits = cap;
    if (want > 1) p.ws = ws;
  }
  if (want < 1) want = 1;
  {
    const int quant = knob<K_WG_QUANT>();
    const int64_t hi_cap = p.ws ? (want * 2 < cap_splits ? want * 2 : cap_splits) : want;
    if (quant && dma && want > 1) {
      const int64_t slots = 256 * (tm == 2 ? 2 : 3);
      int64_t best = want;
      double best_cost = 1e30;
      for (int64_t sp = want / 2 > 1 ? want / 2 : 1; sp <= hi_cap && sp <= cdiv64(p.M, 256); ++sp) {
        if (p.ws && sp * slab > ws_floats) break;
        const int64_t ch = cdiv64(cdiv64(p.M, sp), 64) * 64, real = cdiv64(p.M, ch);
        const double rounds = (double)((tiles * real + slots - 1) / slots);
        const double cost = rounds * ((double)(ch / 64) + 8.0) + 0.02 * (double)real;
        if (cost < best_cost) { best_cost = cost; best = sp; }
      }
      want = best;
    }
  }
  p.chunk = cdiv64(cdiv64(p.M, want), 64) * 64;
  int64_t splits = cdiv64(p.M, p.chunk);
  const int slot = usseg_prof_start(2, s);
  const dim3 grid((unsigned)splits, (unsigned)(p.mtiles * p.ntiles), (unsigned)ntaps);
  const int dbg = knob<K_WGRAD_DEBUG>();
  if (dbg) fprintf(stderr, "[wgrad] M %lld (B %d Hg %d Wg %d) Ma %d Nb %d taps %d tm %d splits %lld chunk %lld slab %s asy %d bsy %d lda %d ldb %d\n", (long long)p.M, p.B, p.Hg, p.Wg,
                   p.Ma, p.Nb, ntaps, tm, (long long)splits, (long long)p.chunk, p.ws ? "yes" : "no", p.asy, p.bsy, p.lda, p.ldb);
  {
    const int pow2_env = knob<K_WGRAD_POW2>();
    auto lg = [](int v) { int l = 0; while ((1 << l) < v) ++l; return (1 << l) == v ? l : -1; };
    p.lw = pow2_env ? lg(p.Wg) : -1;
    p.lh = pow2_env ? lg(p.Hg) : -1;
    if (p.lw < 0 || p.lh < 0) p.lw = p.lh = -1;
  }
  const int xcd_env = knob<K_WGRAD_XCD>();
  p.xcd_remap = dma && xcd_env && p.nb2 <= 0 && (int64_t)splits * p.mtiles * p.ntiles * ntaps < (1ll << 20) && (p.mtiles * p.ntiles * ntaps > 1);
  if (dma) {
    if (tm == 2) wgrad_dma_launch_t<2, 2>(p, grid, s);
    else wgrad_dma_launch_t<1, 3>(p, grid, s);
  } else hipLaunchKernelGGL(wgrad_kernel, grid, dim3(256), 0, s, p);
  if (p.ws) usseg_launch_wgrad_finish(p.ws, (int)splits, slab, p.out, p.map, p.Ma, p.Nb, s);
  usseg_prof_stop(2, slot, s);
  return usseg_check_launch("wgrad");
}

int conv2d_wgrad_impl(const UssegConvDesc* d, const void* x, const void* dy, float* dw, const UssegWgradDst* dst, float* ws, int64_t ws_floats,
                      const UssegTapMask& mask, usseg_stream_t stream) {
  USSEG_CHECK_ARG(d && x && dy && (dw || dst), "null pointer");
  WgMap map;
  USSEG_CHECK_ARG(wg_map_fill(map, dst), "wgrad: bad destination map (1..4 blocks, non-null dst)");
  USSEG_CHECK_ARG(d->Cin % 8 == 0 && d->Cout % 8 == 0 && d->ldx % 8 == 0 && d->ldy % 8 == 0, "channels must be multiples of 8");
  USSEG_CHECK_ARG(d->ksize == 1 || d->ksize == 3, "conv ksize must be 1 or 3");
  if (d->ksize == 3) {
    const WgHaloGeom g = wgrad_halo_geom(*d, x, dy, dw, map, mask);
    if (usseg_try_launch_wgrad_halo(&g, 1, ws, ws_floats, (hipStream_t)stream)) return usseg_check_launch("wgrad_halo");
  }
  WgradParams p = {};
  p.map = map;
  p.a = (const bf16_t*)x; p.b = (const bf16_t*)dy; p.out = dw;
  p.B = d->B; p.Hg = d->H; p.Wg = d->W; p.M = (int64_t)d->B * d->H * d->W;
  p.Ha = d->H; p.Wa = d->W; p.lda = d->ldx; p.asy = p.asx = 1;
  p.Hb = d->H; p.Wb = d->W; p.ldb = d->ldy; p.bsy = p.bsx = 1;
  p.Ma = d->Cin; p.Nb = d->Cout;
  const int k = d->ksize, half = k / 2;
  for (int kh = 0; kh < k; ++kh)
    for (int kw = 0; kw < k; ++kw) {
      int t = kh * k + kw;
      p.ady[t] = (int16_t)((kh - half) * d->dilation); p.adx[t] = (int16_t)((kw - half) * d->dilation);
      p.bdy[t] = 0; p.bdx[t] = 0;
    }
  return launch_wgrad(p, k * k, ws, ws_floats, (hipStream_t)stream);
}

extern "C" int usseg_conv2d_wgrad(const UssegConvDesc* d, const void* x, const void* dy, float* dw, float* ws, int64_t ws_floats,
                                  usseg_stream_t stream) {
  USSEG_CHECK_ARG(dw, "null pointer");
  return conv2d_wgrad_impl(d, x, dy, dw, nullptr, ws, ws_floats, {}, stream);
}
extern "C" int usseg_conv2d_wgrad_mapped(const UssegConvDesc* d, const void* x, const void* dy, const UssegWgradDst* dst, float* ws,
                                         int64_t ws_floats, usseg_stream_t stream) {
  USSEG_CHECK_ARG(dst, "null destination map");
  return conv2d_wgrad_impl(d, x, dy, nullptr, dst, ws, ws_floats, {}, stream);
}

extern "C" int usseg_conv2d_wgrad_multi(int32_t njobs, const UssegWgradJob* jobs, float* ws, int64_t ws_floats, usseg_stream_t stream) {
  USSEG_CHECK_ARG(jobs && njobs >= 1 && njobs <= 4, "wgrad multi: 1 <= njobs <= 4");
  for (int j = 0; j < njobs; ++j) USSEG_CHECK_ARG(jobs[j].x && jobs[j].dy && (jobs[j].dw || jobs[j].dst), "wgrad multi: null pointer");
  WgHaloGeom g[4];
  bool halo = njobs > 1;
  for (int j = 0; j < njobs && halo; ++j) {
    WgMap map;
    halo = jobs[j].desc.ksize == 3 && wg_map_fill(map, jobs[j].dst);
    if (halo) g[j] = wgrad_halo_geom(jobs[j].desc, jobs[j].x, jobs[j].dy, jobs[j].dw, map);
  }
  if (halo && usseg_try_launch_wgrad_halo(g, njobs, ws, ws_floats, (hipStream_t)stream)) return usseg_check_launch("wgrad_halo_multi");
  for (int j = 0; j < njobs; ++j) {
    int rc = conv2d_wgrad_impl(&jobs[j].desc, jobs[j].x, jobs[j].dy, jobs[j].dst ? nullptr : jobs[j].dw, jobs[j].dst, ws, ws_floats, {}, stream);
    if (rc) return rc;
  }
  return USSEG_OK;
}

static int tconv2d_wgrad_impl(const UssegConvDesc* d, const void* x, const void* dy, float* dw, const UssegWgradDst* dst, float* ws,
                              int64_t ws_floats, usseg_stream_t stream) {
  USSEG_CHECK_ARG(d && x && dy && (dw || dst), "null pointer");
  WgMap map;
  USSEG_CHECK_ARG(wg_map_fill(map, dst), "wgrad: bad destination map (1..4 blocks, non-null dst)");
  USSEG_CHECK_ARG(d->Cin % 8 == 0 && d->Cout % 8 == 0 && d->ldx % 8 == 0 && d->ldy % 8 == 0, "channels must be multiples of 8");
  USSEG_CHECK_ARG(d->ksize == 3 || d->ksize == 4, "tconv ksize must be 3 or 4");
  const int k = d->ksize, pad = (k == 4) ? 1 : 0;
  WgradParams p = {};
  p.B = d->B; p.Hg = d->H; p.Wg = d->W; p.M = (int64_t)d->B * d->H * d->W;
  if (!dst) {
    p.a = (const bf16_t*)x; p.b = (const bf16_t*)dy; p.out = dw;
    p.Ha = d->H; p.Wa = d->W; p.lda = d->ldx; p.asy = p.asx = 1;
    p.Hb = 2 * d->H; p.Wb = 2 * d->W; p.ldb = d->ldy; p.bsy = p.bsx = 2;
    p.Ma = d->Cin; p.Nb = d->Cout;
    for (int kh = 0; kh < k; ++kh)
      for (int kw = 0; kw < k; ++kw) {
        int t = kh * k + kw;
        p.ady[t] = 0; p.adx[t] = 0;
        p.bdy[t] = (int16_t)(kh - pad); p.bdx[t] = (int16_t)(kw - pad);
      }
  } else {
    p.a = (const bf16_t*)dy; p.b = (const bf16_t*)x; p.out = nullptr;
    p.Ha = 2 * d->H; p.Wa = 2 * d->W; p.lda = d->ldy; p.asy = p.asx = 2;
    p.Hb = d->H; p.Wb = d->W; p.ldb = d->ldx; p.bsy = p.bsx = 1;
    p.Ma = d->Cout; p.Nb = d->Cin;
    for (int kh = 0; kh < k; ++kh)
      for (int kw = 0; kw < k; ++kw) {
        int t = kh * k + kw;
        p.ady[t] = (int16_t)(kh - pad); p.adx[t] = (int16_t)(kw - pad);
        p.bdy[t] = 0; p.bdx[t] = 0;
      }
    for (int b = 0; b < map.nblocks; ++b) {
      WgBlock u = map.blk[b];
      map.blk[b].sI = u.sO; map.blk[b].sO = u.sI;
      map.blk[b].i_off = u.o_off; map.blk[b].o_off = u.i_off;
      map.blk[b].ni = u.no; map.blk[b].no = u.ni;
    }
    if (usseg_try_launch_tconv_wgrad_halo((const bf16_t*)x, (const bf16_t*)dy, map, d->B, d->H, d->W, d->Cin, d->Cout, d->ldx, d->ldy, k, ws,
                                          ws_floats, (hipStream_t)stream))
      return usseg_check_launch("tconv_wgrad_halo");
  }
  p.map = map;
  return launch_wgrad(p, k * k, ws, ws_floats, (hipStream_t)stream);
}
extern "C" int usseg_tconv2d_wgrad(const UssegConvDesc* d, const void* x, const void* dy, float* dw, usseg_stream_t stream) {
  USSEG_CHECK_ARG(dw, "null pointer");
  return tconv2d_wgrad_impl(d, x, dy, dw, nullptr, nullptr, 0, stream);
}
extern "C" int usseg_tconv2d_wgrad_mapped(const UssegConvDesc* d, const void* x, const void* dy, const UssegWgradDst* dst, float* ws,
                                          int64_t ws_floats, usseg_stream_t stream) {
  USSEG_CHECK_ARG(dst, "null destination map");
  return tconv2d_wgrad_impl(d, x, dy, nullptr, dst, ws, ws_floats, stream);
}

extern "C" int usseg_gemm_tn_batched(const UssegGemmDesc* d, const void* a, const void* b, float* out, usseg_stream_t stream) {
  USSEG_CHECK_ARG(d && a && b && out, "null pointer");
  USSEG_CHECK_ARG(d->M > 0 && d->N > 0 && d->K > 0 && d->M % 8 == 0 && d->N % 8 == 0 && d->ldx % 8 == 0 && d->ldw % 8 == 0,
                  "gemm_tn: M, N, lda, ldb must be multiples of 8");
  USSEG_CHECK_ARG(d->nb1 > 0 && d->nb2 > 0 && (int64_t)d->nb1 * d->nb2 < 65536, "gemm_tn: bad batch");
  WgradParams p = {};
  p.a = (const bf16_t*)a; p.b = (const bf16_t*)b; p.out = out;
  p.B = 1; p.Hg = 1; p.Wg = d->K; p.M = d->K;
  p.Ha = 1; p.Wa = d->K; p.lda = d->ldx; p.asy = p.asx = 1;
  p.Hb = 1; p.Wb = d->K; p.ldb = d->ldw; p.bsy = p.bsx = 1;
  p.Ma = d->M; p.Nb = d->N;
  p.nb2 = d->nb2; p.as1 = d->xs1; p.as2 = d->xs2; p.bs1 = d->ws1; p.bs2 = d->ws2; p.os1 = d->ys1; p.os2 = d->ys2;
  p.mtiles = (p.Ma + 63) / 64;
  p.ntiles = (p.Nb + 63) / 64;
  p.chunk = ((d->K + 63) / 64) * 64;
  p.ntaps = 1;
  const int slot = usseg_prof_start(2, (hipStream_t)stream);
  const int dma_env = knob<K_WGRAD_DMA>();
  const bool dma = dma_env && d->K < (1 << 23) && (int64_t)d->K * d->ldx * 2 < 0x7fff0000ll && (int64_t)d->K * d->ldw * 2 < 0x7fff0000ll &&
                   (d->xs1 | d->xs2 | d->ws1 | d->ws2) % 8 == 0;
  const dim3 grid(1, (unsigned)(p.mtiles * p.ntiles), (unsigned)(d->nb1 * d->nb2));
  if (dma) wgrad_dma_launch_t<1, 3>(p, grid, (hipStream_t)stream);
  else hipLaunchKernelGGL(wgrad_kernel, grid, dim3(256), 0, (hipStream_t)stream, p);
  usseg_prof_stop(2, slot, (hipStream_t)stream);
  return usseg_check_launch("gemm_tn_batched");
}
```

### ultrasound_modeling_amd/csrc/wgrad_halo.hip

```cpp
#include "common.h"

struct WgHaloParams {
  const bf16_t* x;
  const bf16_t* dy;
  float* out;
  float* ws;
  int32_t B, H, W, d, Hl, Wl, PH, PW, NV;
  int32_t tiles_x, tiles_per_v, npatches, ngroups, groups_per_block;
  int32_t ldx, lddy, Ma, Nb, ntiles_n;
  int32_t mask_ch;
  uint16_t tapmask[4];
  int32_t xvd, xvH, xvW, xva, xvb;
  int32_t yvd, yvH, yvW, yva, yvb;
};

struct WgHaloMulti {
  WgHaloParams job[4];
  int32_t xcd_remap;
};

template <int WVM, int WM, int WN, bool PF, int NTG, bool MASKED>
__global__ __launch_bounds__(256 * NTG, NTG == 1 ? 2 : 1) void wgrad_halo_kernel(const WgHaloMulti P) {
  constexpr int NTHR = 256 * NTG, TPG = NTG == 1 ? 9 : 5;
  int bx = blockIdx.x, by = blockIdx.y, bz = blockIdx.z;
  if (P.xcd_remap) {
    const int gx = gridDim.x, gy = gridDim.y, gz = gridDim.z, total = gx * gy * gz;
    const int L = bx + gx * (by + gy * bz);
    const int c = L & 7, q = total >> 3, r = total & 7;
    const int item = c * q + (c < r ? c : r) + (L >> 3);
    const int u = __builtin_amdgcn_readfirstlane(fdiv(item, fdiv_rcp(gy)));
    by = item - u * gy;
    bx = __builtin_amdgcn_readfirstlane(fdiv(u, fdiv_rcp(gz)));
    bz = u - bx * gz;
  }
  const WgHaloParams& p = P.job[bz];
  constexpr int MAXHP = 288;
  constexpr int WVN = 4 / WVM;
  constexpr int BMc = 16 * WM * WVM, BNc = 16 * WN * WVN;
  constexpr int XS = BMc + 16, YS = BNc == 16 ? 48 : BNc + 16;
  constexpr int XCH = BMc / 8, YCH = BNc / 8;
  constexpr int X_IT = (MAXHP * XCH + NTHR - 1) / NTHR, Y_IT = (128 * YCH + NTHR - 1) / NTHR;
  __shared__ __attribute__((aligned(16))) bf16_t lds_x[MAXHP * XS];
  __shared__ __attribute__((aligned(16))) bf16_t lds_y[128 * YS];
  constexpr int TB = NTHR / 8;
  __shared__ __attribute__((aligned(16))) int s_tab[TB][8][8];

  const int tid = threadIdx.x, lane = tid & 63, wv = (tid >> 6) & 3, tg = tid >> 8;
  const int t0 = tg * TPG;
  const int HW2 = p.PW + 2, HPP = (p.PH + 2) * HW2, NHP = p.NV * HPP;
  const int rps = 16 / p.PW, spp = (p.PH * p.PW) >> 4;
  const float r_hpp = fdiv_rcp(HPP), r_hw2 = fdiv_rcp(HW2), r_spp = fdiv_rcp(spp), r_pw = fdiv_rcp(p.PW), r_tpv = fdiv_rcp(p.tiles_per_v),
              r_tx = fdiv_rcp(p.tiles_x), r_dd = fdiv_rcp(p.d * p.d), r_d = fdiv_rcp(p.d);
  int mt, nt;
  fdivmod(by, p.ntiles_n, fdiv_rcp(p.ntiles_n), mt, nt);
  const int m0 = mt * BMc, n0 = nt * BNc;

  int x_geo[X_IT];
#pragma unroll
  for (int it = 0; it < X_IT; ++it) {
    int idx = tid + NTHR * it;
    int hp = idx / XCH;
    x_geo[it] = -1;
    if (hp < NHP) {
      int pi, rem, hy, hx;
      fdivmod(hp, HPP, r_hpp, pi, rem);
      fdivmod(rem, HW2, r_hw2, hy, hx);
      x_geo[it] = (pi << 16) | (hy << 8) | hx;
    }
  }
  int y_geo[Y_IT];
#pragma unroll
  for (int it = 0; it < Y_IT; ++it) {
    int idx = tid + NTHR * it;
    int pk = (idx / YCH) & 127;
    int s = pk >> 4, pl = pk & 15;
    int pi, sl, r, c;
    fdivmod(s, spp, r_spp, pi, sl);
    fdivmod(pl, p.PW, r_pw, r, c);
    y_geo[it] = (pi << 16) | ((sl * rps + r) << 8) | c;
  }
  const int xq = tid % XCH, yq = tid % YCH;
  const bool x_cok = (m0 + xq * 8) < p.Ma, y_cok = (n0 + yq * 8) < p.Nb;
  int x_rel[X_IT], y_rel[Y_IT];
#pragma unroll
  for (int it = 0; it < X_IT; ++it) {
    const int hy = (x_geo[it] >> 8) & 255, hx = x_geo[it] & 255;
    x_rel[it] = __mul24(__mul24(__mul24(p.xvd, hy), p.xvW) + __mul24(p.xvd, hx), p.ldx) + m0 + xq * 8;
  }
#pragma unroll
  for (int it = 0; it < Y_IT; ++it) {
    const int row = (y_geo[it] >> 8) & 255, col = y_geo[it] & 255;
    y_rel[it] = __mul24(__mul24(__mul24(p.yvd, row), p.yvW) + __mul24(p.yvd, col), p.lddy) + n0 + yq * 8;
  }

  const int g = lane >> 4, li = lane & 15, tq = li >> 2, tp = li & 3;
  const int wm = wv / WVN, wn = wv % WVN;
  int xb[4][2], yb[4][2];
#pragma unroll
  for (int ks = 0; ks < 4; ++ks)
#pragma unroll
    for (int h = 0; h < 2; ++h) {
      int pk = 32 * ks + 16 * h + 4 * g + tq;
      int s = pk >> 4, pl = pk & 15;
      int pi, sl, r, c;
      fdivmod(s, spp, r_spp, pi, sl);
      fdivmod(pl, p.PW, r_pw, r, c);
      xb[ks][h] = (pi * HPP + (sl * rps + r) * HW2 + c) * XS + wm * 16 * WM + 4 * tp;
      yb[ks][h] = pk * YS + wn * 16 * WN + 4 * tp;
    }

  f32x4_t acc[TPG][WM][WN];
#pragma unroll
  for (int t = 0; t < TPG; ++t)
#pragma unroll
    for (int i = 0; i < WM; ++i)
#pragma unroll
      for (int j = 0; j < WN; ++j) acc[t][i][j] = (f32x4_t){0.f, 0.f, 0.f, 0.f};

  typedef __attribute__((ext_vector_type(8))) short s16x8_t;
  auto tr8 = [&](const bf16_t* base, int a0, int a1) -> bf16x8_t {
    s16x4_t lo = __builtin_amdgcn_ds_read_tr16_b64_v4i16((s16x4_t __attribute__((address_space(3)))*)(base + a0));
    s16x4_t hi = __builtin_amdgcn_ds_read_tr16_b64_v4i16((s16x4_t __attribute__((address_space(3)))*)(base + a1));
    s16x8_t v = {lo[0], lo[1], lo[2], lo[3], hi[0], hi[1], hi[2], hi[3]};
    return __builtin_bit_cast(bf16x8_t, v);
  };

  const int g_begin = bx * p.groups_per_block;
  int g_end = g_begin + p.groups_per_block;
  if (g_end > p.ngroups) g_end = p.ngroups;

  auto fill_batch = [&](int grp0) {
    const int gi = tid >> 3, pi = tid & 7;
    int (*tab)[8] = s_tab[gi];
    if (pi < p.NV) {
      const int tid = pi;
      int gp = (grp0 + gi) * p.NV + pi;
      int valid = gp < p.npatches && (grp0 + gi) < g_end;
      int gpc = valid ? gp : 0;
      int v, tt, ty, tx, b, ab, la, lb;
      fdivmod(gpc, p.tiles_per_v, r_tpv, v, tt);
      fdivmod(tt, p.tiles_x, r_tx, ty, tx);
      fdivmod(v, p.d * p.d, r_dd, b, ab);
      fdivmod(ab, p.d, r_d, la, lb);
      const int ly0 = __mul24(ty, p.PH), lx0 = __mul24(tx, p.PW);
      tab[tid][0] = __mul24(__mul24(__mul24(b, p.xvH) + p.xva + la + __mul24(p.xvd, ly0 - 1), p.xvW) + p.xvb + lb + __mul24(p.xvd, lx0 - 1), p.ldx);
      tab[tid][1] = __mul24(__mul24(__mul24(b, p.yvH) + p.yva + la + __mul24(p.yvd, ly0), p.yvW) + p.yvb + lb + __mul24(p.yvd, lx0), p.lddy);
      tab[tid][2] = valid ? ly0 - 1 : -(1 << 24);
      tab[tid][3] = lx0 - 1;
      tab[tid][4] = valid;
    }
  };
  const bool nv1 = p.NV == 1;
  auto load_xy = [&](int (*tab)[8], uint4 (&rx)[X_IT], uint4 (&ry)[Y_IT], uint32_t& mx, uint32_t& my) {
    mx = my = 0u;
    int4 ex[X_IT];
    int yorg[Y_IT], yval[Y_IT];
    if (nv1) {
      const int4 e = *reinterpret_cast<const int4*>(tab[0]);
      const int v = tab[0][4];
#pragma unroll
      for (int it = 0; it < X_IT; ++it) ex[it] = e;
#pragma unroll
      for (int it = 0; it < Y_IT; ++it) { yorg[it] = e.y; yval[it] = v; }
    } else {
#pragma unroll
      for (int it = 0; it < X_IT; ++it) {
        const int geo = x_geo[it] < 0 ? 0 : x_geo[it];
        ex[it] = *reinterpret_cast<const int4*>(tab[geo >> 16]);
      }
#pragma unroll
      for (int it = 0; it < Y_IT; ++it) {
        const int* pt = tab[y_geo[it] >> 16];
        yorg[it] = pt[1];
        yval[it] = pt[4];
      }
    }
#pragma unroll
    for (int it = 0; it < X_IT; ++it) asm volatile("" : "+v"(ex[it].x), "+v"(ex[it].z), "+v"(ex[it].w));
#pragma unroll
    for (int it = 0; it < Y_IT; ++it) asm volatile("" : "+v"(yorg[it]), "+v"(yval[it]));
#pragma unroll
    for (int it = 0; it < X_IT; ++it) {
      const int geo = x_geo[it] < 0 ? 0 : x_geo[it];
      const int ly = ex[it].z + ((geo >> 8) & 255), lx = ex[it].w + (geo & 255);
      const bool ok = (x_geo[it] >= 0) & x_cok & ((unsigned)ly < (unsigned)p.Hl) & ((unsigned)lx < (unsigned)p.Wl);
      rx[it] = *reinterpret_cast<const uint4*>(p.x + (ok ? ex[it].x + x_rel[it] : 0));
      mx |= (ok ? 1u : 0u) << it;
    }
#pragma unroll
    for (int it = 0; it < Y_IT; ++it) {
      const bool ok = (tid + NTHR * it < 128 * YCH) & y_cok & (yval[it] != 0);
      ry[it] = *reinterpret_cast<const uint4*>(p.dy + (ok ? yorg[it] + y_rel[it] : 0));
      my |= (ok ? 1u : 0u) << it;
    }
  };
  const uint32_t tmask = (MASKED && p.mask_ch) ? p.tapmask[n0 / p.mask_ch] : 0x1ffu;
  int toff_t[TPG];
#pragma unroll
  for (int tt = 0; tt < TPG; ++tt) {
    const int t = (t0 + tt) < 9 ? (t0 + tt) : 8;
    toff_t[tt] = __builtin_amdgcn_readfirstlane(((t / 3) * HW2 + (t % 3)) * XS);
  }
  const bool last_ok = __builtin_amdgcn_readfirstlane(t0 + TPG - 1) < 9;
  auto compute = [&]() {
    bf16x8_t af[2][WM], bfr[2][WN];
    auto load_b = [&](int ks, bf16x8_t (&b)[WN]) {
#pragma unroll
      for (int j = 0; j < WN; ++j) b[j] = tr8(lds_y, yb[ks][0] + 16 * j, yb[ks][1] + 16 * j);
    };
    auto load_a = [&](int ks, int tt, bf16x8_t (&a)[WM]) {
#pragma unroll
      for (int i = 0; i < WM; ++i) a[i] = tr8(lds_x, xb[ks][0] + toff_t[tt] + 16 * i, xb[ks][1] + toff_t[tt] + 16 * i);
    };
    load_b(0, bfr[0]);
    load_a(0, 0, af[0]);
#pragma unroll
    for (int st = 0; st < 4 * TPG; ++st) {
      const int ks = st / TPG, tt = st - ks * TPG;
      if (st + 1 < 4 * TPG) {
        const int ks1 = (st + 1) / TPG, tt1 = (st + 1) - ks1 * TPG;
        if (tt1 == 0) load_b(ks1, bfr[ks1 & 1]);
        load_a(ks1, tt1, af[(st + 1) & 1]);
      }
      __builtin_amdgcn_sched_barrier(0);
      const bool skip = (NTG > 1 && tt == TPG - 1 && !last_ok) ||
                        (MASKED && !((tmask >> (t0 + tt)) & 1u));
      if (!skip) {
#pragma unroll
        for (int i = 0; i < WM; ++i)
#pragma unroll
          for (int j = 0; j < WN; ++j)
            acc[tt][i][j] = __builtin_amdgcn_mfma_f32_16x16x32_bf16(bfr[ks & 1][j], af[st & 1][i], acc[tt][i][j], 0, 0, 0);
      }
      __builtin_amdgcn_sched_barrier(0);
    }
  };

  if (!PF) {
    for (int grp = g_begin; grp < g_end; ++grp) {
      const int rel = grp - g_begin;
      if ((rel & (TB - 1)) == 0) fill_batch(grp);
      __syncthreads();
      uint4 rx[X_IT], ry[Y_IT];
      uint32_t mx, my;
      load_xy(s_tab[rel & (TB - 1)], rx, ry, mx, my);
#pragma unroll
      for (int it = 0; it < X_IT; ++it)
        if (x_geo[it] >= 0)
          *reinterpret_cast<uint4*>(&lds_x[((tid + NTHR * it) / XCH) * XS + xq * 8]) = (mx >> it) & 1u ? rx[it] : make_uint4(0, 0, 0, 0);
#pragma unroll
      for (int it = 0; it < Y_IT; ++it)
        if (tid + NTHR * it < 128 * YCH)
          *reinterpret_cast<uint4*>(&lds_y[((tid + NTHR * it) / YCH) * YS + yq * 8]) = (my >> it) & 1u ? ry[it] : make_uint4(0, 0, 0, 0);
      __syncthreads();
      compute();
    }
  } else {
    uint4 rx[X_IT], ry[Y_IT];
    uint32_t mx = 0u, my = 0u;
    if (g_begin < g_end) {
      fill_batch(g_begin);
      __syncthreads();
      load_xy(s_tab[0], rx, ry, mx, my);
    }
    for (int grp = g_begin; grp < g_end; ++grp) {
      const int rel1 = grp + 1 - g_begin;
      int (*nxt)[8] = s_tab[rel1 & (TB - 1)];
#pragma unroll
      for (int it = 0; it < X_IT; ++it)
        if (x_geo[it] >= 0)
          *reinterpret_cast<uint4*>(&lds_x[((tid + NTHR * it) / XCH) * XS + xq * 8]) = (mx >> it) & 1u ? rx[it] : make_uint4(0, 0, 0, 0);
#pragma unroll
      for (int it = 0; it < Y_IT; ++it)
        if (tid + NTHR * it < 128 * YCH)
          *reinterpret_cast<uint4*>(&lds_y[((tid + NTHR * it) / YCH) * YS + yq * 8]) = (my >> it) & 1u ? ry[it] : make_uint4(0, 0, 0, 0);
      const bool more = grp + 1 < g_end;
      if (more && (rel1 & (TB - 1)) == 0) fill_batch(grp + 1);
      __syncthreads();
      if (more) {
        load_xy(nxt, rx, ry, mx, my);
      }
      compute();
      __syncthreads();
    }
  }

  float* dst = p.ws ? p.ws + (int64_t)bx * 9 * p.Ma * p.Nb : p.out;
  const bool vec_ok = (p.Nb & 3) == 0;
#pragma unroll
  for (int tt = 0; tt < TPG; ++tt)
#pragma unroll
    for (int i = 0; i < WM; ++i)
#pragma unroll
      for (int j = 0; j < WN; ++j) {
        const int t = t0 + tt;
        if (NTG > 1 && t >= 9) continue;
        const int m = m0 + wm * 16 * WM + i * 16 + li;
        const int n = n0 + wn * 16 * WN + j * 16 + g * 4;
        if (m >= p.Ma || n >= p.Nb) continue;
        float* q = dst + ((int64_t)t * p.Ma + m) * p.Nb + n;
        if (p.ws && vec_ok && n + 3 < p.Nb) {
          *reinterpret_cast<float4*>(q) = make_float4(acc[tt][i][j][0], acc[tt][i][j][1], acc[tt][i][j][2], acc[tt][i][j][3]);
        } else {
#pragma unroll
          for (int r = 0; r < 4; ++r)
            if (n + r < p.Nb) {
              if (p.ws) q[r] = acc[tt][i][j][r];
              else atomicAdd(q + r, acc[tt][i][j][r]);
            }
        }
      }
}

int usseg_try_launch_wgrad_halo(const WgHaloGeom* gm, int njobs, float* ws, int64_t ws_floats, hipStream_t s) {
  const int disabled = knob<K_NO_HALO>();
  if (disabled || njobs < 1 || njobs > 4) return 0;
  WgHaloMulti P;
  const int Ma = gm[0].Ma, Nb = gm[0].Nb;
  auto shape_of = [](int ma, int nb) { return (ma <= 32 && nb <= 32) ? 1 : (nb <= 16 ? 2 : (nb <= 32 ? 3 : 0)); };
  auto tiles_of = [&](int ma, int nb) {
    const int sh = shape_of(ma, nb), bm = sh == 1 ? 32 : 64, bn = sh == 0 ? 64 : (sh == 2 ? 16 : 32);
    return ((ma + bm - 1) / bm) * ((nb + bn - 1) / bn);
  };
  int64_t slab_max = 0, slab_sum = 0;
  for (int j = 0; j < njobs; ++j) {
    const WgHaloGeom& q = gm[j];
    if (q.B != gm[0].B || q.H != gm[0].H || q.W != gm[0].W) return 0;
    if (shape_of(q.Ma, q.Nb) != shape_of(Ma, Nb) || tiles_of(q.Ma, q.Nb) != tiles_of(Ma, Nb)) return 0;
    if ((q.Ma != Ma || q.Nb != Nb) && (q.mask.group_ch || q.tconv_cls >= 0)) return 0;
    slab_sum += (int64_t)9 * q.Ma * q.Nb;
    if ((int64_t)9 * q.Ma * q.Nb > slab_max) slab_max = (int64_t)9 * q.Ma * q.Nb;
    const int d = q.d;
    if (d < 1 || q.H % d || q.W % d) return 0;
    const int Hl = q.H / d, Wl = q.W / d;
    int PW;
    if (Wl % 16 == 0) PW = 16;
    else if (Wl == 8 || Wl == 4) PW = Wl;
    else return 0;
    int PH = 128 / PW;
    if (PH > Hl) PH = Hl;
    if (Hl % PH || (PH * PW) % 16) return 0;
    const int NV = 128 / (PH * PW);
    if (NV * (PH + 2) * (PW + 2) > 288) return 0;
    WgHaloParams& p = P.job[j];
    p = {};
    p.x = q.x; p.dy = q.dy; p.out = q.out;
    p.B = q.B; p.H = q.H; p.W = q.W; p.d = d; p.Hl = Hl; p.Wl = Wl; p.PH = PH; p.PW = PW; p.NV = NV;
    p.tiles_x = Wl / PW;
    p.tiles_per_v = (Hl / PH) * p.tiles_x;
    p.npatches = q.B * d * d * p.tiles_per_v;
    if (q.tconv_cls >= 0) {
      p.xvd = 2; p.xvH = 2 * q.H; p.xvW = 2 * q.W; p.xva = q.tconv_cls >> 1; p.xvb = q.tconv_cls & 1;
      p.yvd = 1; p.yvH = q.H; p.yvW = q.W; p.yva = p.yvb = 0;
      p.mask_ch = 1 << 30;
      p.tapmask[0] = (uint16_t)q.tapmask;
    } else {
      p.xvd = p.yvd = d; p.xvH = p.yvH = q.H; p.xvW = p.yvW = q.W; p.xva = p.xvb = p.yva = p.yvb = 0;
    }
    p.ngroups = (p.npatches + NV - 1) / NV;
    p.ldx = q.ldx; p.lddy = q.lddy; p.Ma = q.Ma; p.Nb = q.Nb;
    if (p.ngroups != P.job[0].ngroups) return 0;
    if ((int64_t)q.B * p.xvH * p.xvW * q.ldx >= (1ll << 31) || (int64_t)q.B * p.yvH * p.yvW * q.lddy >= (1ll << 31)) return 0;
    if ((int64_t)q.B * p.xvH * p.xvW >= (1ll << 23) || (int64_t)q.B * p.yvH * p.yvW >= (1ll << 23) || p.npatches >= (1 << 20)) return 0;
  }
  if (ws) ws = usseg_defer_wgrad_ws(s, ws, ws_floats, &ws_floats);
  int shape = 0;
  if (Ma <= 32 && Nb <= 32) shape = 1;
  else if (Nb <= 16) shape = 2;
  else if (Nb <= 32) shape = 3;
  const int bm = shape == 1 ? 32 : 64, bn = shape == 0 ? 64 : (shape == 2 ? 16 : 32);
  const int tm = (Ma + bm - 1) / bm;
  const int ntn = (Nb + bn - 1) / bn;
  const int tiles = tm * ntn;
  const int ngroups = P.job[0].ngroups;
  const int64_t slab = slab_max;
  int64_t in_bytes = 0;
  for (int j = 0; j < njobs; ++j) in_bytes += (int64_t)gm[j].B * gm[j].H * gm[j].W * (gm[j].Ma + gm[j].Nb) * 2;
  in_bytes /= njobs;
  const int64_t slab_bytes = slab * 4;
  const int wg_target = knob<K_WG_TARGET>();
  int splits = (wg_target + tiles * njobs - 1) / (tiles * njobs);
  int max_splits = (ngroups + 1) / 2;
  const int slab_cap = knob<K_SLAB_CAP>();
  const int64_t traffic_cap = slab_cap * in_bytes / slab_bytes < 4 ? 4 : slab_cap * in_bytes / slab_bytes;
  if (max_splits > traffic_cap) max_splits = (int)traffic_cap;
  if (!ws) max_splits = (ngroups + 15) / 16;
  else if ((int64_t)max_splits * slab_sum > ws_floats) max_splits = (int)(ws_floats / slab_sum);
  if (splits > max_splits) splits = max_splits;
  if (splits < 1) splits = 1;
  {
    const int quant = knob<K_WG_QUANT>();
    if (quant && max_splits > 1) {
      const int slots = 256 * (shape == 0 ? 1 : 2);
      const int64_t tj = (int64_t)tiles * njobs;
      int best = splits;
      double best_cost = 1e30;
      const int lo = splits / 2 > 1 ? splits / 2 : 1, hi = splits * 2 < max_splits ? splits * 2 : max_splits;
      for (int sp = lo; sp <= hi; ++sp) {
        const int g = (ngroups + sp - 1) / sp;
        const int real = (ngroups + g - 1) / g;
        const double rounds = (double)((tj * real + slots - 1) / slots);
        const double cost = rounds * (g + 3.0) + 0.02 * real;
        if (cost < best_cost) { best_cost = cost; best = sp; }
      }
      splits = best;
    }
  }
  bool mapped = false;
  for (int j = 0; j < njobs; ++j) mapped = mapped || gm[j].map.nblocks;
  const bool use_ws = ws && (splits > 1 || mapped) && (int64_t)splits * slab_sum <= ws_floats;
  if (mapped && !use_ws) return 0;
  const int gpb = (ngroups + splits - 1) / splits;
  splits = (ngroups + gpb - 1) / gpb;
  {
    int64_t off = 0;
    for (int j = 0; j < njobs; ++j) {
      P.job[j].ntiles_n = (gm[j].Nb + bn - 1) / bn;
      P.job[j].groups_per_block = gpb;
      P.job[j].ws = use_ws ? ws + off : nullptr;
      off += (int64_t)splits * 9 * gm[j].Ma * gm[j].Nb;
    }
  }
  const UssegTapMask& qm = gm[0].mask;
  const bool masked = qm.group_ch != 0 || gm[0].tconv_cls >= 0;
  if (qm.group_ch) {
    if (njobs != 1 || qm.group_ch % bn) return 0;
    P.job[0].mask_ch = qm.group_ch;
    for (int c = 0; c < 4; ++c) P.job[0].tapmask[c] = qm.mask[c];
  }
  const dim3 grid(splits, tiles, njobs);
  const int xcd_env = knob<K_WGHALO_XCD>();
  P.xcd_remap = xcd_env && tiles * njobs > 1 && (int64_t)splits * tiles * njobs < (1ll << 20);
  const int dbg = knob<K_WGRAD_DEBUG>();
  if (dbg) fprintf(stderr, "[wgrad_halo] B %d H %d W %d d %d Ma %d Nb %d jobs %d shape %d tiles %d ngroups %d splits %d gpb %d max_splits %d traffic_cap %lld slab_MB %.2f in_MB %.2f\n",
                   gm[0].B, gm[0].H, gm[0].W, gm[0].d, Ma, Nb, njobs, shape, tiles, ngroups, splits, gpb, max_splits, (long long)traffic_cap, slab_bytes / 1e6, in_bytes / 1e6);
  const int slot = usseg_prof_start(2, s);
  const int pf = knob<K_WGRAD_PF>();
  if (shape == 1) {
    if (pf) { if (masked) hipLaunchKernelGGL((wgrad_halo_kernel<2, 1, 1, true, 1, true>), grid, dim3(256), 0, s, P); else hipLaunchKernelGGL((wgrad_halo_kernel<2, 1, 1, true, 1, false>), grid, dim3(256), 0, s, P); }
    else { if (masked) hipLaunchKernelGGL((wgrad_halo_kernel<2, 1, 1, false, 1, true>), grid, dim3(256), 0, s, P); else hipLaunchKernelGGL((wgrad_halo_kernel<2, 1, 1, false, 1, false>), grid, dim3(256), 0, s, P); }
  } else if (shape == 2) {
    if (pf) { if (masked) hipLaunchKernelGGL((wgrad_halo_kernel<4, 1, 1, true, 1, true>), grid, dim3(256), 0, s, P); else hipLaunchKernelGGL((wgrad_halo_kernel<4, 1, 1, true, 1, false>), grid, dim3(256), 0, s, P); }
    else { if (masked) hipLaunchKernelGGL((wgrad_halo_kernel<4, 1, 1, false, 1, true>), grid, dim3(256), 0, s, P); else hipLaunchKernelGGL((wgrad_halo_kernel<4, 1, 1, false, 1, false>), grid, dim3(256), 0, s, P); }
  } else if (shape == 3) {
    if (pf) { if (masked) hipLaunchKernelGGL((wgrad_halo_kernel<4, 1, 2, true, 1, true>), grid, dim3(256), 0, s, P); else hipLaunchKernelGGL((wgrad_halo_kernel<4, 1, 2, true, 1, false>), grid, dim3(256), 0, s, P); }
    else { if (masked) hipLaunchKernelGGL((wgrad_halo_kernel<4, 1, 2, false, 1, true>), grid, dim3(256), 0, s, P); else hipLaunchKernelGGL((wgrad_halo_kernel<4, 1, 2, false, 1, false>), grid, dim3(256), 0, s, P); }
  } else {
    const int tg8 = knob<K_WGRAD_8W>();
    if (tg8) { if (masked) hipLaunchKernelGGL((wgrad_halo_kernel<2, 2, 2, true, 2, true>), grid, dim3(512), 0, s, P); else hipLaunchKernelGGL((wgrad_halo_kernel<2, 2, 2, true, 2, false>), grid, dim3(512), 0, s, P); }
    else { if (masked) hipLaunchKernelGGL((wgrad_halo_kernel<2, 2, 2, false, 1, true>), grid, dim3(256), 0, s, P); else hipLaunchKernelGGL((wgrad_halo_kernel<2, 2, 2, false, 1, false>), grid, dim3(256), 0, s, P); }
  }
  if (use_ws)
    for (int j = 0; j < njobs; ++j) usseg_launch_wgrad_finish(P.job[j].ws, splits, (int64_t)9 * gm[j].Ma * gm[j].Nb, gm[j].out, gm[j].map, gm[j].Ma, gm[j].Nb, s);
  usseg_prof_stop(2, slot, s);
  return 1;
}

int usseg_try_launch_tconv_wgrad_halo(const bf16_t* x, const bf16_t* dy, const WgMap& map, int B, int H, int W, int Cin, int Cout, int ldx,
                                      int lddy, int k, float* ws, int64_t ws_floats, hipStream_t s) {
  const int enabled = knob<K_TCONV_HALO>();
  if (!enabled || map.nblocks < 1 || (k != 3 && k != 4)) return 0;
  const int pad = k == 4 ? 1 : 0;
  WgHaloGeom g[4];
  for (int c = 0; c < 4; ++c) {
    const int a = c >> 1, b = c & 1;
    uint32_t mask = 0;
    for (int th = 0; th < 3; ++th)
      for (int tw = 0; tw < 3; ++tw) {
        const int kh = a + pad - 2 + 2 * th, kw = b + pad - 2 + 2 * tw;
        if (kh >= 0 && kh < k && kw >= 0 && kw < k) mask |= 1u << (3 * th + tw);
      }
    g[c] = {dy, x, nullptr, map, B, H, W, 1, Cout, Cin, lddy, ldx};
    g[c].tconv_cls = c;
    g[c].tapmask = mask;
    g[c].map.tapmask = mask;
    for (int i = 0; i < map.nblocks; ++i) {
      WgBlock& u = g[c].map.blk[i];
      const int64_t sk = map.blk[i].sT;
      u.dst = map.blk[i].dst + ((int64_t)(a + pad - 2) * k + (b + pad - 2)) * sk;
      u.sTr = 2 * k * sk;
      u.sT = 2 * sk;
    }
  }
  return usseg_try_launch_wgrad_halo(g, 4, ws, ws_floats, s);
}
```

### ultrasound_modeling_amd/knobs.py

```python
from __future__ import annotations

import os

KNOBS = {
    "USSEG_LIB":                ("str",    None,  "path of a diagnostic build of the same sources to load instead of the in-tree library"),
    "USSEG_SIDE_STREAM":        ("flag",   0,     "weight gradients fork to a side stream per launch inside an overlap region"),
    "USSEG_DEFER":              ("flag",   1,     "defer the finishing reductions to the end of the region (0: finish after each producer)"),
    "USSEG_LAZY_WGRAD":         ("flag",   1,     "lazy weight gradients: queued and run on the side stream beside the backward-data chain"),
    "USSEG_FUSE_LN_RES":        ("flag",   1,     "LayerNorm backward + residual add in one pass (transformer blocks)"),
    "USSEG_ENC_LAZY":           ("optint", None,  "bit mask of the ResNest stages whose weight gradients are lazy (unset: 12, or 0 in front of a ViT)"),
    "USSEG_FOLD_BN":            ("flag",   1,     "inference BatchNorm folded into the producing conv's packed weights"),
    "USSEG_FUSED_CARDINAL":     ("flag",   1,     "cardinal group + shortcut of a stage as one launch"),
    "USSEG_FUSED_CARDINAL_BWD": ("flag",   1,     "its backward chain + the shortcut norm's backward as one launch"),
    "USSEG_CARD_BWD_MAX_PX":    ("int",    32768, "most pixels of a stage for the fused cardinal backward"),
    "USSEG_LN_PAIR":            ("flag",   1,     "shortcut norm backward + conv2_bn backward of the large stages in one launch"),
    "USSEG_FUSED_STEM_BWD":     ("flag",   1,     "stem backward-data fused with the norm / activation backward in front"),
    "USSEG_STEM_WGRAD_MERGE":   ("flag",   1,     "the stem's three weight gradients in one multi-job launch"),
    "USSEG_FUSED_STEM":         ("flag",   1,     "the stem (three convs, two norms, pool) as one launch"),
    "USSEG_MERGED_DGRAD":       ("flag",   1,     "one backward-data GEMM for a stage's grouped 1x1 and shortcut 1x1"),
    "USSEG_FUSED_DGRAD":        ("flag",   1,     "the DecoderBlock's four branch backward-data passes as one launch"),
    "USSEG_BRANCH4":            ("flag",   1,     "the DecoderBlock's 1x1 branch as a fourth job of the dilated branches' launch"),
    "USSEG_QUAD_UP":            ("flag",   0,     "the decoder's transposed convs in quad (parity-class) form"),
    "USSEG_QUAD_HEAD":          ("flag",   1,     "the <= 4-class head's transposed conv in quad form (read at construction)"),
    "USSEG_QUAD_TCONV":         ("flag",   0,     "Arch A's inner transposed convs in quad form (read at construction)"),
    "USSEG_STAGE_LAZY":         ("flag",   1,     "Arch A: per-stage lazy weight gradients"),
    "USSEG_FUSED_HEAD":         ("flag",   1,     "head conv + softmax + loss as one launch"),
    "USSEG_VIT_LAZY":           ("str",    "enc", "lazy weight gradients of the ViT: whole encoder (enc), per block (block), or 0"),
    "USSEG_FUSED_ATTN":         ("flag",   1,     "train-step attention on the fused kernels (head size 128)"),
    "USSEG_SWIN_LAZY":          ("flag",   1,     "Swin: per-block lazy weight gradients"),
    "USSEG_DIST_BACKEND":       ("str",    None,  "torch.distributed backend (unset: nccl with a GPU, else gloo)"),
    "USSEG_DP_CHUNKS":          ("int",    0,     "chunks of the pipelined gradient exchange (0 or 1: one exchange)"),
}


def get(name: str):
    rule, default, _ = KNOBS[name]
    v = os.environ.get(name)
    if rule == "flag":
        return bool(default) if v is None else v != "0"
    if v is None:
        return default
    return v if rule == "str" else int(v)
```

Before: 5815.

## Add cost-model planner for weight-gradient tile shape and split-K count

Pulls the per-tap and halo weight-gradient tiling and split decisions out into planner functions. The per-tap planner adds a calibrated cost model that searches tile size and split count for single-tap cases and switches away from the channel-class rule only when the estimated gain clears a margin. The halo path gets a matching planner, and both planners are exposed through C entry points with a force knob for sweeps and tests. The cost constants are hand-calibrated, so plans for some shapes may change and could regress.

```diff
diff --git a/include/usseg.h b/include/usseg.h
--- a/include/usseg.h
+++ b/include/usseg.h
@@ -83,6 +83,27 @@
   const UssegWgradDst* dst;
 } UssegWgradJob;
 int usseg_conv2d_wgrad_multi(int32_t njobs, const UssegWgradJob* jobs, float* ws, int64_t ws_floats, usseg_stream_t stream);
+
+typedef struct UssegWgradPlanGeom {
+  int32_t B, H, W, d;
+  int32_t Ma, Nb;
+  int32_t group_ch, reserved;
+} UssegWgradPlanGeom;
+typedef struct UssegWgradPlan {
+  int32_t ok;
+  int32_t shape;
+  int32_t tile_m, tile_n;
+  int32_t tiles;
+  int32_t splits;
+  int32_t per_block;
+  int32_t slots;
+  int32_t max_splits;
+  float cost_us;
+  int64_t workgroups;
+  int64_t slab_bytes;
+} UssegWgradPlan;
+int usseg_wgrad_halo_plan(int32_t njobs, const UssegWgradPlanGeom* jobs, int64_t ws_floats, int32_t mapped, int64_t force, UssegWgradPlan* out);
+int usseg_wgrad_pertap_plan(int64_t M, int32_t Ma, int32_t Nb, int32_t ntaps, int64_t ws_floats, int64_t force, UssegWgradPlan* out);
 
 int usseg_defer_begin(usseg_stream_t stream, float* reduce_ws, int64_t reduce_floats, float* wgrad_ws, int64_t wgrad_floats);
 int usseg_defer_flush(usseg_stream_t stream);
diff --git a/ultrasound_modeling_amd/_lib.py b/ultrasound_modeling_amd/_lib.py
--- a/ultrasound_modeling_amd/_lib.py
+++ b/ultrasound_modeling_amd/_lib.py
@@ -40,6 +40,15 @@
 
 class WgradJob(C.Structure):
     _fields_ = [("desc", ConvDesc), ("x", c_vp), ("dy", c_vp), ("dw", c_vp), ("dst", P_WgradDst)]
+
+
+class WgradPlanGeom(C.Structure):
+    _fields_ = [("B", c_i32), ("H", c_i32), ("W", c_i32), ("d", c_i32), ("Ma", c_i32), ("Nb", c_i32), ("group_ch", c_i32), ("reserved", c_i32)]
+
+
+class WgradPlan(C.Structure):
+    _fields_ = [("ok", c_i32), ("shape", c_i32), ("tile_m", c_i32), ("tile_n", c_i32), ("tiles", c_i32), ("splits", c_i32), ("per_block", c_i32),
+                ("slots", c_i32), ("max_splits", c_i32), ("cost_us", c_f32), ("workgroups", c_i64), ("slab_bytes", c_i64)]
 
 
 class AugSample(C.Structure):
@@ -151,6 +160,8 @@
     "usseg_tconv2d_wgrad_mapped": (C.c_int, [P(ConvDesc), c_vp, c_vp, P(WgradDst), c_vp, c_i64, c_vp]),
     "usseg_conv2d_dgrad_branches": (C.c_int, [P(ConvDesc), c_i32, c_vp, c_vp, c_vp, c_i32, c_vp, c_vp, c_vp, c_i32, c_vp, c_vp]),
     "usseg_conv2d_wgrad_multi": (C.c_int, [c_i32, c_vp, c_vp, c_i64, c_vp]),
+    "usseg_wgrad_halo_plan": (C.c_int, [c_i32, c_vp, c_i64, c_i32, c_i64, P(WgradPlan)]),
+    "usseg_wgrad_pertap_plan": (C.c_int, [c_i64, c_i32, c_i32, c_i32, c_i64, c_i64, P(WgradPlan)]),
     "usseg_conv2d_fwd_multi": (C.c_int, [c_i32, c_vp, c_vp]),
     "usseg_conv2d_dgrad_multi": (C.c_int, [c_i32, c_vp, c_vp]),
     "usseg_tconv2d_fwd": (C.c_int, [P(ConvDesc), c_vp, c_vp, c_vp, c_vp, c_vp]),
diff --git a/ultrasound_modeling_amd/csrc/knobs.h b/ultrasound_modeling_amd/csrc/knobs.h
--- a/ultrasound_modeling_amd/csrc/knobs.h
+++ b/ultrasound_modeling_amd/csrc/knobs.h
@@ -42,6 +42,7 @@
   X(K_WGD_CAP,            "USSEG_WGD_CAP",            INT,     4,     ONCE,     "per-tap wgrad: slab traffic cap, in multiples of the operand bytes") \
   X(K_WG_QUANT,           "USSEG_WG_QUANT",           INT,     1,     ONCE,     "0: no wave-quantisation search of the split count (both wgrad kernels)") \
   X(K_WGRAD_DEBUG,        "USSEG_WGRAD_DEBUG",        PRESENT, 0,     ONCE,     "print every weight-gradient plan to stderr")               \
+  X(K_WGRAD_PLAN,         "USSEG_WGRAD_PLAN",         INT,     0,     ONCE,     "force weight-gradient plans: splits*100 + per-tap tile*10 + halo shape (0: planner, 9: channel-class rule)") \
   X(K_WGRAD_POW2,         "USSEG_WGRAD_POW2",         INT,     1,     ONCE,     "0: no shift decode of power-of-two grids")                 \
   X(K_WGRAD_XCD,          "USSEG_WGRAD_XCD",          INT,     1,     ONCE,     "0: no XCD-aware item order in the per-tap wgrad")          \
   X(K_WG_TARGET,          "USSEG_WG_TARGET",          INT,     256,   ONCE,     "halo wgrad: workgroups the split-K aims for")              \
diff --git a/ultrasound_modeling_amd/csrc/wgrad.hip b/ultrasound_modeling_amd/csrc/wgrad.hip
--- a/ultrasound_modeling_amd/csrc/wgrad.hip
+++ b/ultrasound_modeling_amd/csrc/wgrad.hip
@@ -330,64 +330,167 @@
   hipLaunchKernelGGL((wgrad_dma_kernel<TM, NSTAGE>), grid, dim3(256), dyn, s, p, 1.0f / (float)(p.Hg * p.Wg), 1.0f / (float)p.Wg);
 }
 
+struct WgTapPlanIn {
+  int64_t M;
+  int Ma, Nb, ntaps;
+  bool dma;
+  int64_t ws_floats;
+};
+struct WgTapPlan {
+  int tm;
+  int64_t splits, chunk, cap_splits;
+  bool slabs;
+  double cost_us;
+};
+static inline int64_t tap_tiles(const WgTapPlanIn& in, int tm) {
+  const int bt = 64 * tm;
+  return (int64_t)((in.Ma + bt - 1) / bt) * ((in.Nb + bt - 1) / bt) * in.ntaps;
+}
+static inline int64_t tap_slots(int tm) { return 256 * (tm == 2 ? 2 : 3); }
+static const double kTapStepUs[2][3] = {{0, 0.42, 0.68}, {0, 0.87, 1.42}};
+static const double kTapFixedUs[2][3] = {{0, 8.1, 8.0}, {0, 3.1, 4.5}};
+static const double kTapSlabUsPerMB[2] = {0.53, 0.39};
+static const double kTapMarginUs = 1.5, kTapMarginRel = 0.10;
+static double tap_cost_us(const WgTapPlanIn& in, int tm, int64_t sp, bool slabs, int64_t* chunk_out = nullptr, int64_t* real_out = nullptr) {
+  const int64_t ch = cdiv64(cdiv64(in.M, sp), 64) * 64, real = cdiv64(in.M, ch);
+  const double rounds = (double)((tap_tiles(in, tm) * real + tap_slots(tm) - 1) / tap_slots(tm));
+  if (chunk_out) *chunk_out = ch;
+  if (real_out) *real_out = real;
+  const int k = in.ntaps > 1;
+  return rounds * ((double)(ch / 64) * kTapStepUs[k][tm] + kTapFixedUs[k][tm]) + (slabs ? (double)real * in.ntaps * in.Ma * in.Nb * 4 * 1e-6 * kTapSlabUsPerMB[k] : 0.0);
+}
+
+static int64_t tap_cap_splits(const WgTapPlanIn& in) {
+  const int64_t slab = (int64_t)in.ntaps * in.Ma * in.Nb, in_bytes = in.M * (in.Ma + in.Nb) * 2;
+  const int slab_cap = knob<K_WGD_CAP>();
+  int64_t cap = slab_cap * in_bytes / (slab * 4);
+  if (cap < 4) cap = 4;
+  if (cap > in.ws_floats / slab) cap = in.ws_floats / slab;
+  return cap;
+}
+
+static void tap_plan_by_class(const WgTapPlanIn& in, int tm_forced, WgTapPlan* out) {
+  int tm = 1;
+  if (in.dma && in.Ma > 64 && in.Nb > 64) tm = 2;
+  if (in.dma && tm_forced) tm = tm_forced;
+  const int64_t tiles = tap_tiles(in, tm);
+  const int wg_target = knob<K_WGD_TARGET>();
+  int64_t want = (wg_target + tiles - 1) / tiles;
+  const int64_t max_splits = cdiv64(in.M, 256);
+  if (want > max_splits) want = max_splits;
+  if (want < 1) want = 1;
+  const int64_t slab = (int64_t)in.ntaps * in.Ma * in.Nb;
+  bool slabs = false;
+  int64_t cap_splits = 1;
+  if (in.ws_floats && want > 1) {
+    const int64_t cap = tap_cap_splits(in);
+    if (want > cap) want = cap;
+    cap_splits = cap;
+    if (want > 1) slabs = true;
+  }
+  if (want < 1) want = 1;
+  {
+    const int quant = knob<K_WG_QUANT>();
+    const int64_t hi_cap = slabs ? (want * 2 < cap_splits ? want * 2 : cap_splits) : want;
+    if (quant && in.dma && want > 1) {
+      const int64_t slots = tap_slots(tm);
+      int64_t best = want;
+      double best_cost = 1e30;
+      for (int64_t sp = want / 2 > 1 ? want / 2 : 1; sp <= hi_cap && sp <= cdiv64(in.M, 256); ++sp) {
+        if (slabs && sp * slab > in.ws_floats) break;
+        const int64_t ch = cdiv64(cdiv64(in.M, sp), 64) * 64, real = cdiv64(in.M, ch);
+        const double rounds = (double)((tiles * real + slots - 1) / slots);
+        const double cost = rounds * ((double)(ch / 64) + 8.0) + 0.02 * (double)real;
+        if (cost < best_cost) { best_cost = cost; best = sp; }
+      }
+      want = best;
+    }
+  }
+  out->tm = tm; out->slabs = slabs; out->cap_splits = cap_splits;
+  out->cost_us = tap_cost_us(in, tm, want, slabs, &out->chunk, &out->splits);
+}
+
+static int64_t tap_wgs(const WgTapPlanIn& in, int tm, int64_t sp) {
+  const int64_t ch = cdiv64(cdiv64(in.M, sp), 64) * 64;
+  return cdiv64(in.M, ch) * tap_tiles(in, tm);
+}
+static int64_t tap_most_in_round(const WgTapPlanIn& in, int tm, int64_t max_splits) {
+  int64_t most = 0;
+  for (int64_t sp = 1; sp <= max_splits; ++sp) {
+    const int64_t w = tap_wgs(in, tm, sp);
+    if (w <= tap_slots(tm) && w > most) most = w;
+  }
+  return most;
+}
+static bool tap_fills(const WgTapPlanIn& in, int tm, int64_t sp, int64_t most_in_round) {
+  const int64_t w = tap_wgs(in, tm, sp);
+  return w >= tap_slots(tm) || w >= most_in_round;
+}
+
+static void tap_plan(const WgTapPlanIn& in, int64_t force, WgTapPlan* out) {
+  const int tm_env = (int)knob<K_WGRAD_TM>();
+  WgTapPlan base;
+  tap_plan_by_class(in, tm_env, &base);
+  *out = base;
+  const int ftm = (int)(force / 10 % 10);
+  int64_t fsplits = force / 100;
+  if (ftm == 9 || !in.dma || !in.ws_floats) return;
+  if (in.ntaps > 1 && !ftm && !fsplits) return;
+  if (!ftm && !fsplits && cdiv64(in.M, 64) * tap_tiles(in, base.tm) < 256) return;
+  const int64_t slab = (int64_t)in.ntaps * in.Ma * in.Nb;
+  int64_t hard = cdiv64(in.M, 256);
+  if (hard > in.ws_floats / slab) hard = in.ws_floats / slab;
+  if (hard < 1) hard = 1;
+  if (fsplits > hard) fsplits = hard;
+  const int64_t cap = base.cap_splits > 1 ? base.cap_splits : tap_cap_splits(in);
+  const bool forced = ftm || fsplits;
+  const int64_t most_sp = cap < hard ? cap : hard;
+  double best_cost = 1e30, same_cost = 1e30;
+  WgTapPlan same = base;
+  for (int tm = 1; tm <= 2; ++tm) {
+    if ((ftm == 1 || ftm == 2) && tm != ftm) continue;
+    if (!ftm && tm_env && tm != tm_env) continue;
+    const int64_t lo = fsplits ? fsplits : 1, hi = fsplits ? fsplits : most_sp;
+    const int64_t most = forced ? 0 : tap_most_in_round(in, tm, most_sp);
+    for (int64_t sp = lo; sp <= hi; ++sp) {
+      int64_t ch, real;
+      const double c = tap_cost_us(in, tm, sp, sp > 1, &ch, &real) + 1e-3 * (double)real;
+      if (real > 1 && real * slab > in.ws_floats) continue;
+      if (!forced && !tap_fills(in, tm, sp, most)) continue;
+      WgTapPlan q = base;
+      q.tm = tm; q.splits = real; q.chunk = ch; q.slabs = real > 1; q.cost_us = c;
+      if (c < best_cost) { best_cost = c; *out = q; }
+      if (tm == base.tm && c < same_cost) { same_cost = c; same = q; }
+    }
+  }
+  if (best_cost >= 1e30) { *out = base; return; }
+  if (forced) return;
+  if (base.cost_us - out->cost_us < (kTapMarginUs > kTapMarginRel * base.cost_us ? kTapMarginUs : kTapMarginRel * base.cost_us))
+    *out = tap_fills(in, base.tm, base.splits, tap_most_in_round(in, base.tm, most_sp)) ? base : same;
+}
+
 static int launch_wgrad(WgradParams& p, int ntaps, float* ws, int64_t ws_floats, hipStream_t s) {
   const int dma_env = knob<K_WGRAD_DMA>();
   const bool dma = dma_env && p.nb2 <= 0 && p.M < (1 << 24) && (int64_t)p.Hg * p.Wg < (1 << 23) && (int64_t)p.B * p.Ha * p.Wa < (1 << 24) && (int64_t)p.B * p.Hb * p.Wb < (1 << 24) &&
                    (int64_t)p.B * p.Ha * p.Wa * p.lda * 2 < 0x7fff0000ll &&
                    (int64_t)p.B * p.Hb * p.Wb * p.ldb * 2 < 0x7fff0000ll && p.lda % 8 == 0 && p.ldb % 8 == 0;
-  const int tm_env = knob<K_WGRAD_TM>();
-  int tm = 1;
-  if (dma && p.Ma > 64 && p.Nb > 64) tm = 2;
-  if (dma && tm_env) tm = tm_env;
-  const int bt = 64 * tm;
+  if (ws) ws = usseg_defer_wgrad_ws(s, ws, ws_floats, &ws_floats);
+  const WgTapPlanIn in = {p.M, p.Ma, p.Nb, ntaps, dma, ws ? ws_floats : 0};
+  WgTapPlan plan;
+  tap_plan(in, knob<K_WGRAD_PLAN>(), &plan);
+  const int tm = plan.tm, bt = 64 * tm;
   p.mtiles = (p.Ma + bt - 1) / bt;
   p.ntiles = (p.Nb + bt - 1) / bt;
   p.ntaps = ntaps;
-  int64_t tiles = (int64_t)p.mtiles * p.ntiles * ntaps;
-  const int wg_target = knob<K_WGD_TARGET>();
-  const int slab_cap = knob<K_WGD_CAP>();
-  int64_t want = (wg_target + tiles - 1) / tiles;
-  int64_t max_splits = cdiv64(p.M, 256);
-  if (want > max_splits) want = max_splits;
-  if (want < 1) want = 1;
   const int64_t slab = (int64_t)ntaps * p.Ma * p.Nb;
-  p.ws = nullptr;
-  int64_t cap_splits = 1;
-  if (ws) ws = usseg_defer_wgrad_ws(s, ws, ws_floats, &ws_floats);
-  if (ws && want > 1) {
-    const int64_t in_bytes = p.M * (p.Ma + p.Nb) * 2;
-    int64_t cap = slab_cap * in_bytes / (slab * 4);
-    if (cap < 4) cap = 4;
-    if (cap > ws_floats / slab) cap = ws_floats / slab;
-    if (want > cap) want = cap;
-    cap_splits = cap;
-    if (want > 1) p.ws = ws;
-  }
-  if (want < 1) want = 1;
-  {
-    const int quant = knob<K_WG_QUANT>();
-    const int64_t hi_cap = p.ws ? (want * 2 < cap_splits ? want * 2 : cap_splits) : want;
-    if (quant && dma && want > 1) {
-      const int64_t slots = 256 * (tm == 2 ? 2 : 3);
-      int64_t best = want;
-      double best_cost = 1e30;
-      for (int64_t sp = want / 2 > 1 ? want / 2 : 1; sp <= hi_cap && sp <= cdiv64(p.M, 256); ++sp) {
-        if (p.ws && sp * slab > ws_floats) break;
-        const int64_t ch = cdiv64(cdiv64(p.M, sp), 64) * 64, real = cdiv64(p.M, ch);
-        const double rounds = (double)((tiles * real + slots - 1) / slots);
-        const double cost = rounds * ((double)(ch / 64) + 8.0) + 0.02 * (double)real;
-        if (cost < best_cost) { best_cost = cost; best = sp; }
-      }
-      want = best;
-    }
-  }
-  p.chunk = cdiv64(cdiv64(p.M, want), 64) * 64;
-  int64_t splits = cdiv64(p.M, p.chunk);
+  p.ws = plan.slabs ? ws : nullptr;
+  p.chunk = plan.chunk;
+  const int64_t splits = plan.splits;
   const int slot = usseg_prof_start(2, s);
   const dim3 grid((unsigned)splits, (unsigned)(p.mtiles * p.ntiles), (unsigned)ntaps);
   const int dbg = knob<K_WGRAD_DEBUG>();
-  if (dbg) fprintf(stderr, "[wgrad] M %lld (B %d Hg %d Wg %d) Ma %d Nb %d taps %d tm %d splits %lld chunk %lld slab %s asy %d bsy %d lda %d ldb %d\n", (long long)p.M, p.B, p.Hg, p.Wg,
-                   p.Ma, p.Nb, ntaps, tm, (long long)splits, (long long)p.chunk, p.ws ? "yes" : "no", p.asy, p.bsy, p.lda, p.ldb);
+  if (dbg) fprintf(stderr, "[wgrad] M %lld (B %d Hg %d Wg %d) Ma %d Nb %d taps %d tm %d tile %dx%d splits %lld chunk %lld slab %s slabs_MB %.2f est_us %.1f asy %d bsy %d lda %d ldb %d\n", (long long)p.M, p.B, p.Hg, p.Wg,
+                   p.Ma, p.Nb, ntaps, tm, bt, bt, (long long)splits, (long long)p.chunk, p.ws ? "yes" : "no", p.ws ? splits * slab * 4 / 1e6 : 0.0, plan.cost_us, p.asy, p.bsy, p.lda, p.ldb);
   {
     const int pow2_env = knob<K_WGRAD_POW2>();
     auto lg = [](int v) { int l = 0; while ((1 << l) < v) ++l; return (1 << l) == v ? l : -1; };
@@ -404,6 +507,23 @@
   if (p.ws) usseg_launch_wgrad_finish(p.ws, (int)splits, slab, p.out, p.map, p.Ma, p.Nb, s);
   usseg_prof_stop(2, slot, s);
   return usseg_check_launch("wgrad");
+}
+
+extern "C" int usseg_wgrad_pertap_plan(int64_t M, int32_t Ma, int32_t Nb, int32_t ntaps, int64_t ws_floats, int64_t force, UssegWgradPlan* out) {
+  USSEG_CHECK_ARG(out && M > 0 && Ma > 0 && Nb > 0 && ntaps > 0 && ws_floats >= 0, "wgrad_pertap_plan: bad geometry");
+  *out = {};
+  const WgTapPlanIn in = {M, Ma, Nb, ntaps, true, ws_floats};
+  WgTapPlan plan;
+  tap_plan(in, force < 0 ? knob<K_WGRAD_PLAN>() : force, &plan);
+  out->ok = 1; out->shape = plan.tm; out->tile_m = out->tile_n = 64 * plan.tm;
+  out->tiles = (int32_t)tap_tiles(in, plan.tm); out->splits = (int32_t)plan.splits; out->per_block = (int32_t)(plan.chunk / 64);
+  out->slots = (int32_t)tap_slots(plan.tm);
+  const int64_t cap = ws_floats ? tap_cap_splits(in) : 1, most = cdiv64(M, 256);
+  out->max_splits = (int32_t)(cap < most ? cap : most);
+  out->workgroups = plan.splits * tap_tiles(in, plan.tm);
+  out->slab_bytes = plan.slabs ? plan.splits * (int64_t)ntaps * Ma * Nb * 4 : 0;
+  out->cost_us = (float)plan.cost_us;
+  return USSEG_OK;
 }
 
 int conv2d_wgrad_impl(const UssegConvDesc* d, const void* x, const void* dy, float* dw, const UssegWgradDst* dst, float* ws, int64_t ws_floats,
diff --git a/ultrasound_modeling_amd/csrc/wgrad_halo.hip b/ultrasound_modeling_amd/csrc/wgrad_halo.hip
--- a/ultrasound_modeling_amd/csrc/wgrad_halo.hip
+++ b/ultrasound_modeling_amd/csrc/wgrad_halo.hip
@@ -312,36 +312,187 @@
       }
 }
 
+static bool halo_patch(int H, int W, int d, int* PHo, int* PWo, int* NVo) {
+  if (d < 1 || H % d || W % d) return false;
+  const int Hl = H / d, Wl = W / d;
+  int PW;
+  if (Wl % 16 == 0) PW = 16;
+  else if (Wl == 8 || Wl == 4) PW = Wl;
+  else return false;
+  int PH = 128 / PW;
+  if (PH > Hl) PH = Hl;
+  if (Hl % PH || (PH * PW) % 16) return false;
+  const int NV = 128 / (PH * PW);
+  if (NV * (PH + 2) * (PW + 2) > 288) return false;
+  *PHo = PH; *PWo = PW; *NVo = NV;
+  return true;
+}
+
+static const int kHaloBm[4] = {64, 32, 64, 64}, kHaloBn[4] = {64, 32, 16, 32};
+static inline int halo_slots(int sh) { return 256 * (sh == 0 ? 1 : 2); }
+static inline int halo_class(int ma, int nb) { return (ma <= 32 && nb <= 32) ? 1 : (nb <= 16 ? 2 : (nb <= 32 ? 3 : 0)); }
+static inline int halo_tiles(int sh, int ma, int nb) { return ((ma + kHaloBm[sh] - 1) / kHaloBm[sh]) * ((nb + kHaloBn[sh] - 1) / kHaloBn[sh]); }
+
+struct WgHaloPlanIn {
+  int njobs, Ma[4], Nb[4];
+  int ngroups;
+  int group_ch;
+  int mapped;
+  int64_t in_bytes;
+  int64_t ws_floats;
+};
+struct WgHaloPlan {
+  int shape, tiles, splits, gpb, max_splits;
+  int64_t traffic_cap;
+  double cost_us;
+};
+
+static bool halo_shape_legal(const WgHaloPlanIn& in, int sh) {
+  for (int j = 1; j < in.njobs; ++j)
+    if (halo_tiles(sh, in.Ma[j], in.Nb[j]) != halo_tiles(sh, in.Ma[0], in.Nb[0])) return false;
+  return !(in.group_ch && in.group_ch % kHaloBn[sh]);
+}
+
+static int64_t halo_slab_sum(const WgHaloPlanIn& in) {
+  int64_t v = 0;
+  for (int j = 0; j < in.njobs; ++j) v += (int64_t)9 * in.Ma[j] * in.Nb[j];
+  return v;
+}
+
+static const double kHaloGroupUs[4] = {2.62, 1.78, 2.08, 2.32};
+static const double kHaloFixedUs[4] = {10.5, 6.2, 6.9, 9.7};
+static const double kSlabUsPerMB = 0.23;
+static const double kPlanMarginUs = 2.0, kPlanMarginRel = 0.20;
+static double halo_cost_us(const WgHaloPlanIn& in, int sh, int splits, int* gpb_out = nullptr, int* real_out = nullptr) {
+  const int gpb = (in.ngroups + splits - 1) / splits, real = (in.ngroups + gpb - 1) / gpb;
+  const int64_t wgs = (int64_t)halo_tiles(sh, in.Ma[0], in.Nb[0]) * in.njobs * real;
+  const double rounds = (double)((wgs + halo_slots(sh) - 1) / halo_slots(sh));
+  const bool slabs = in.ws_floats > 0 && (real > 1 || in.mapped);
+  if (gpb_out) *gpb_out = gpb;
+  if (real_out) *real_out = real;
+  return rounds * (gpb * kHaloGroupUs[sh] + kHaloFixedUs[sh]) + (slabs ? real * halo_slab_sum(in) * 4 * 1e-6 * kSlabUsPerMB : 0.0);
+}
+
+static int halo_max_splits(const WgHaloPlanIn& in, int64_t* traffic_cap_out) {
+  int64_t slab_max = 0;
+  for (int j = 0; j < in.njobs; ++j)
+    if ((int64_t)9 * in.Ma[j] * in.Nb[j] > slab_max) slab_max = (int64_t)9 * in.Ma[j] * in.Nb[j];
+  const int slab_cap = knob<K_SLAB_CAP>();
+  const int64_t slab_bytes = slab_max * 4;
+  const int64_t traffic_cap = slab_cap * in.in_bytes / slab_bytes < 4 ? 4 : slab_cap * in.in_bytes / slab_bytes;
+  int max_splits = (in.ngroups + 1) / 2;
+  if (max_splits > traffic_cap) max_splits = (int)traffic_cap;
+  if (!in.ws_floats) max_splits = (in.ngroups + 15) / 16;
+  else if ((int64_t)max_splits * halo_slab_sum(in) > in.ws_floats) max_splits = (int)(in.ws_floats / halo_slab_sum(in));
+  if (traffic_cap_out) *traffic_cap_out = traffic_cap;
+  return max_splits < 1 ? 1 : max_splits;
+}
+
+static bool halo_plan_by_class(const WgHaloPlanIn& in, WgHaloPlan* out) {
+  const int shape = halo_class(in.Ma[0], in.Nb[0]);
+  for (int j = 1; j < in.njobs; ++j)
+    if (halo_class(in.Ma[j], in.Nb[j]) != shape) return false;
+  if (!halo_shape_legal(in, shape)) return false;
+  const int tiles = halo_tiles(shape, in.Ma[0], in.Nb[0]);
+  const int wg_target = knob<K_WG_TARGET>();
+  int splits = (wg_target + tiles * in.njobs - 1) / (tiles * in.njobs);
+  int64_t traffic_cap;
+  const int max_splits = halo_max_splits(in, &traffic_cap);
+  if (splits > max_splits) splits = max_splits;
+  if (splits < 1) splits = 1;
+  {
+    const int quant = knob<K_WG_QUANT>();
+    if (quant && max_splits > 1) {
+      const int slots = halo_slots(shape);
+      const int64_t tj = (int64_t)tiles * in.njobs;
+      int best = splits;
+      double best_cost = 1e30;
+      const int lo = splits / 2 > 1 ? splits / 2 : 1, hi = splits * 2 < max_splits ? splits * 2 : max_splits;
+      for (int sp = lo; sp <= hi; ++sp) {
+        const int g = (in.ngroups + sp - 1) / sp;
+        const int real = (in.ngroups + g - 1) / g;
+        const double rounds = (double)((tj * real + slots - 1) / slots);
+        const double cost = rounds * (g + 3.0) + 0.02 * real;
+        if (cost < best_cost) { best_cost = cost; best = sp; }
+      }
+      splits = best;
+    }
+  }
+  out->shape = shape; out->tiles = tiles; out->max_splits = max_splits; out->traffic_cap = traffic_cap;
+  out->cost_us = halo_cost_us(in, shape, splits, &out->gpb, &out->splits);
+  return true;
+}
+
+static int64_t halo_wgs(const WgHaloPlanIn& in, int sh, int splits) {
+  const int gpb = (in.ngroups + splits - 1) / splits, real = (in.ngroups + gpb - 1) / gpb;
+  return (int64_t)halo_tiles(sh, in.Ma[0], in.Nb[0]) * in.njobs * real;
+}
+static int64_t halo_most_in_round(const WgHaloPlanIn& in, int sh, int max_splits) {
+  int64_t most = 0;
+  for (int sp = 1; sp <= max_splits; ++sp) {
+    const int64_t w = halo_wgs(in, sh, sp);
+    if (w <= halo_slots(sh) && w > most) most = w;
+  }
+  return most;
+}
+static bool halo_fills(const WgHaloPlanIn& in, int sh, int splits, int64_t most_in_round) {
+  const int64_t w = halo_wgs(in, sh, splits);
+  return w >= halo_slots(sh) || w >= most_in_round;
+}
+
+static bool halo_plan(const WgHaloPlanIn& in, int64_t force, WgHaloPlan* out) {
+  WgHaloPlan base;
+  if (!halo_plan_by_class(in, &base)) return false;
+  *out = base;
+  const int fshape = (int)(force % 10), fsplits = (int)(force / 100);
+  if (fshape == 9) return true;
+  if (!fshape && !fsplits && (int64_t)in.ngroups * base.tiles * in.njobs < 256) return true;
+  int hard = (in.ngroups + 1) / 2;
+  if (!in.ws_floats) hard = 1;
+  else if ((int64_t)hard * halo_slab_sum(in) > in.ws_floats) hard = (int)(in.ws_floats / halo_slab_sum(in));
+  if (hard < 1) hard = 1;
+  const bool forced = fshape || fsplits;
+  double best_cost = 1e30, same_cost = 1e30;
+  WgHaloPlan same = base;
+  for (int sh = 0; sh < 4; ++sh) {
+    if (fshape >= 1 && fshape <= 4 && sh != fshape - 1 && halo_shape_legal(in, fshape - 1)) continue;
+    if (!halo_shape_legal(in, sh)) continue;
+    const int lo = fsplits ? (fsplits < hard ? fsplits : hard) : 1, hi = fsplits ? lo : base.max_splits;
+    const int64_t most = forced ? 0 : halo_most_in_round(in, sh, base.max_splits);
+    for (int sp = lo; sp <= hi; ++sp) {
+      int gpb, real;
+      const double c = halo_cost_us(in, sh, sp, &gpb, &real) + 1e-3 * real;
+      if (!forced && !halo_fills(in, sh, real, most)) continue;
+      WgHaloPlan q = base;
+      q.shape = sh; q.tiles = halo_tiles(sh, in.Ma[0], in.Nb[0]); q.splits = real; q.gpb = gpb; q.cost_us = c;
+      if (c < best_cost) { best_cost = c; *out = q; }
+      if (sh == base.shape && c < same_cost) { same_cost = c; same = q; }
+    }
+  }
+  if (best_cost >= 1e30) { *out = base; return true; }
+  if (forced) return true;
+  if (base.cost_us - out->cost_us < (kPlanMarginUs > kPlanMarginRel * base.cost_us ? kPlanMarginUs : kPlanMarginRel * base.cost_us))
+    *out = halo_fills(in, base.shape, base.splits, halo_most_in_round(in, base.shape, base.max_splits)) ? base : same;
+  return true;
+}
+
 int usseg_try_launch_wgrad_halo(const WgHaloGeom* gm, int njobs, float* ws, int64_t ws_floats, hipStream_t s) {
   const int disabled = knob<K_NO_HALO>();
   if (disabled || njobs < 1 || njobs > 4) return 0;
   WgHaloMulti P;
   const int Ma = gm[0].Ma, Nb = gm[0].Nb;
-  auto shape_of = [](int ma, int nb) { return (ma <= 32 && nb <= 32) ? 1 : (nb <= 16 ? 2 : (nb <= 32 ? 3 : 0)); };
-  auto tiles_of = [&](int ma, int nb) {
-    const int sh = shape_of(ma, nb), bm = sh == 1 ? 32 : 64, bn = sh == 0 ? 64 : (sh == 2 ? 16 : 32);
-    return ((ma + bm - 1) / bm) * ((nb + bn - 1) / bn);
-  };
-  int64_t slab_max = 0, slab_sum = 0;
+  WgHaloPlanIn in = {};
+  in.njobs = njobs;
   for (int j = 0; j < njobs; ++j) {
     const WgHaloGeom& q = gm[j];
     if (q.B != gm[0].B || q.H != gm[0].H || q.W != gm[0].W) return 0;
-    if (shape_of(q.Ma, q.Nb) != shape_of(Ma, Nb) || tiles_of(q.Ma, q.Nb) != tiles_of(Ma, Nb)) return 0;
     if ((q.Ma != Ma || q.Nb != Nb) && (q.mask.group_ch || q.tconv_cls >= 0)) return 0;
-    slab_sum += (int64_t)9 * q.Ma * q.Nb;
-    if ((int64_t)9 * q.Ma * q.Nb > slab_max) slab_max = (int64_t)9 * q.Ma * q.Nb;
+    in.Ma[j] = q.Ma; in.Nb[j] = q.Nb;
+    in.in_bytes += (int64_t)q.B * q.H * q.W * (q.Ma + q.Nb) * 2;
     const int d = q.d;
-    if (d < 1 || q.H % d || q.W % d) return 0;
+    int PH, PW, NV;
+    if (!halo_patch(q.H, q.W, d, &PH, &PW, &NV)) return 0;
     const int Hl = q.H / d, Wl = q.W / d;
-    int PW;
-    if (Wl % 16 == 0) PW = 16;
-    else if (Wl == 8 || Wl == 4) PW = Wl;
-    else return 0;
-    int PH = 128 / PW;
-    if (PH > Hl) PH = Hl;
-    if (Hl % PH || (PH * PW) % 16) return 0;
-    const int NV = 128 / (PH * PW);
-    if (NV * (PH + 2) * (PW + 2) > 288) return 0;
     WgHaloParams& p = P.job[j];
     p = {};
     p.x = q.x; p.dy = q.dy; p.out = q.out;
@@ -364,54 +515,19 @@
     if ((int64_t)q.B * p.xvH * p.xvW >= (1ll << 23) || (int64_t)q.B * p.yvH * p.yvW >= (1ll << 23) || p.npatches >= (1 << 20)) return 0;
   }
   if (ws) ws = usseg_defer_wgrad_ws(s, ws, ws_floats, &ws_floats);
-  int shape = 0;
-  if (Ma <= 32 && Nb <= 32) shape = 1;
-  else if (Nb <= 16) shape = 2;
-  else if (Nb <= 32) shape = 3;
-  const int bm = shape == 1 ? 32 : 64, bn = shape == 0 ? 64 : (shape == 2 ? 16 : 32);
-  const int tm = (Ma + bm - 1) / bm;
-  const int ntn = (Nb + bn - 1) / bn;
-  const int tiles = tm * ntn;
-  const int ngroups = P.job[0].ngroups;
-  const int64_t slab = slab_max;
-  int64_t in_bytes = 0;
-  for (int j = 0; j < njobs; ++j) in_bytes += (int64_t)gm[j].B * gm[j].H * gm[j].W * (gm[j].Ma + gm[j].Nb) * 2;
-  in_bytes /= njobs;
-  const int64_t slab_bytes = slab * 4;
-  const int wg_target = knob<K_WG_TARGET>();
-  int splits = (wg_target + tiles * njobs - 1) / (tiles * njobs);
-  int max_splits = (ngroups + 1) / 2;
-  const int slab_cap = knob<K_SLAB_CAP>();
-  const int64_t traffic_cap = slab_cap * in_bytes / slab_bytes < 4 ? 4 : slab_cap * in_bytes / slab_bytes;
-  if (max_splits > traffic_cap) max_splits = (int)traffic_cap;
-  if (!ws) max_splits = (ngroups + 15) / 16;
-  else if ((int64_t)max_splits * slab_sum > ws_floats) max_splits = (int)(ws_floats / slab_sum);
-  if (splits > max_splits) splits = max_splits;
-  if (splits < 1) splits = 1;
-  {
-    const int quant = knob<K_WG_QUANT>();
-    if (quant && max_splits > 1) {
-      const int slots = 256 * (shape == 0 ? 1 : 2);
-      const int64_t tj = (int64_t)tiles * njobs;
-      int best = splits;
-      double best_cost = 1e30;
-      const int lo = splits / 2 > 1 ? splits / 2 : 1, hi = splits * 2 < max_splits ? splits * 2 : max_splits;
-      for (int sp = lo; sp <= hi; ++sp) {
-        const int g = (ngroups + sp - 1) / sp;
-        const int real = (ngroups + g - 1) / g;
-        const double rounds = (double)((tj * real + slots - 1) / slots);
-        const double cost = rounds * (g + 3.0) + 0.02 * real;
-        if (cost < best_cost) { best_cost = cost; best = sp; }
-      }
-      splits = best;
-    }
-  }
   bool mapped = false;
   for (int j = 0; j < njobs; ++j) mapped = mapped || gm[j].map.nblocks;
+  in.in_bytes /= njobs;
+  in.ngroups = P.job[0].ngroups;
+  in.group_ch = gm[0].mask.group_ch;
+  in.mapped = mapped;
+  in.ws_floats = ws ? ws_floats : 0;
+  WgHaloPlan plan;
+  if (!halo_plan(in, knob<K_WGRAD_PLAN>(), &plan)) return 0;
+  const int shape = plan.shape, bn = kHaloBn[shape], tiles = plan.tiles, splits = plan.splits, gpb = plan.gpb, ngroups = in.ngroups;
+  const int64_t slab_sum = halo_slab_sum(in);
   const bool use_ws = ws && (splits > 1 || mapped) && (int64_t)splits * slab_sum <= ws_floats;
   if (mapped && !use_ws) return 0;
-  const int gpb = (ngroups + splits - 1) / splits;
-  splits = (ngroups + gpb - 1) / gpb;
   {
     int64_t off = 0;
     for (int j = 0; j < njobs; ++j) {
@@ -432,8 +548,9 @@
   const int xcd_env = knob<K_WGHALO_XCD>();
   P.xcd_remap = xcd_env && tiles * njobs > 1 && (int64_t)splits * tiles * njobs < (1ll << 20);
   const int dbg = knob<K_WGRAD_DEBUG>();
-  if (dbg) fprintf(stderr, "[wgrad_halo] B %d H %d W %d d %d Ma %d Nb %d jobs %d shape %d tiles %d ngroups %d splits %d gpb %d max_splits %d traffic_cap %lld slab_MB %.2f in_MB %.2f\n",
-                   gm[0].B, gm[0].H, gm[0].W, gm[0].d, Ma, Nb, njobs, shape, tiles, ngroups, splits, gpb, max_splits, (long long)traffic_cap, slab_bytes / 1e6, in_bytes / 1e6);
+  if (dbg) fprintf(stderr, "[wgrad_halo] B %d H %d W %d d %d Ma %d Nb %d jobs %d shape %d tile %dx%d class %d tiles %d ngroups %d splits %d gpb %d max_splits %d traffic_cap %lld slabs_MB %.2f in_MB %.2f est_us %.1f\n",
+                   gm[0].B, gm[0].H, gm[0].W, gm[0].d, Ma, Nb, njobs, shape, kHaloBm[shape], bn, halo_class(Ma, Nb), tiles, ngroups, splits, gpb, plan.max_splits,
+                   (long long)plan.traffic_cap, use_ws ? splits * slab_sum * 4 / 1e6 : 0.0, in.in_bytes / 1e6, plan.cost_us);
   const int slot = usseg_prof_start(2, s);
   const int pf = knob<K_WGRAD_PF>();
   if (shape == 1) {
@@ -484,3 +601,38 @@
   }
   return usseg_try_launch_wgrad_halo(g, 4, ws, ws_floats, s);
 }
+
+extern "C" int usseg_wgrad_halo_plan(int32_t njobs, const UssegWgradPlanGeom* jobs, int64_t ws_floats, int32_t mapped, int64_t force, UssegWgradPlan* out) {
+  USSEG_CHECK_ARG(jobs && out && njobs >= 1 && njobs <= 4 && ws_floats >= 0, "wgrad_halo_plan: 1 <= njobs <= 4, non-null pointers");
+  *out = {};
+  WgHaloPlanIn in = {};
+  in.njobs = njobs;
+  for (int j = 0; j < njobs; ++j) {
+    const UssegWgradPlanGeom& q = jobs[j];
+    USSEG_CHECK_ARG(q.B > 0 && q.H > 0 && q.W > 0 && q.Ma > 0 && q.Nb > 0, "wgrad_halo_plan: bad geometry");
+    int PH, PW, NV;
+    if (q.B != jobs[0].B || q.H != jobs[0].H || q.W != jobs[0].W || !halo_patch(q.H, q.W, q.d, &PH, &PW, &NV)) return USSEG_OK;
+    if ((q.Ma != jobs[0].Ma || q.Nb != jobs[0].Nb) && q.group_ch) return USSEG_OK;
+    const int ngroups = (q.B * q.d * q.d * ((q.H / q.d) / PH) * ((q.W / q.d) / PW) + NV - 1) / NV;
+    if (j && ngroups != in.ngroups) return USSEG_OK;
+    in.ngroups = ngroups;
+    in.Ma[j] = q.Ma; in.Nb[j] = q.Nb;
+    in.in_bytes += (int64_t)q.B * q.H * q.W * (q.Ma + q.Nb) * 2;
+  }
+  in.in_bytes /= njobs;
+  in.group_ch = jobs[0].group_ch;
+  in.mapped = mapped;
+  in.ws_floats = ws_floats;
+  if (in.group_ch && njobs != 1) return USSEG_OK;
+  WgHaloPlan plan;
+  if (!halo_plan(in, force < 0 ? knob<K_WGRAD_PLAN>() : force, &plan)) return USSEG_OK;
+  const bool slabs = ws_floats > 0 && (plan.splits > 1 || mapped);
+  if (mapped && !slabs) return USSEG_OK;
+  out->ok = 1; out->shape = plan.shape; out->tile_m = kHaloBm[plan.shape]; out->tile_n = kHaloBn[plan.shape];
+  out->tiles = plan.tiles; out->splits = plan.splits; out->per_block = plan.gpb; out->slots = halo_slots(plan.shape);
+  out->max_splits = plan.max_splits;
+  out->workgroups = (int64_t)plan.splits * plan.tiles * njobs;
+  out->slab_bytes = slabs ? plan.splits * halo_slab_sum(in) * 4 : 0;
+  out->cost_us = (float)plan.cost_us;
+  return USSEG_OK;
+}
diff --git a/ultrasound_modeling_amd/knobs.py b/ultrasound_modeling_amd/knobs.py
--- a/ultrasound_modeling_amd/knobs.py
+++ b/ultrasound_modeling_amd/knobs.py
@@ -28,6 +28,7 @@
     "USSEG_VIT_LAZY":           ("str",    "enc", "lazy weight gradients of the ViT: whole encoder (enc), per block (block), or 0"),
     "USSEG_FUSED_ATTN":         ("flag",   1,     "train-step attention on the fused kernels (head size 128)"),
     "USSEG_SWIN_LAZY":          ("flag",   1,     "Swin: per-block lazy weight gradients"),
+    "USSEG_WGRAD_PLAN":         ("int",    0,     "weight-gradient plan override of the kernel library (csrc/knobs.h), read here by the sweep tool and the plan tests"),
     "USSEG_DIST_BACKEND":       ("str",    None,  "torch.distributed backend (unset: nccl with a GPU, else gloo)"),
     "USSEG_DP_CHUNKS":          ("int",    0,     "chunks of the pipelined gradient exchange (0 or 1: one exchange)"),
 }
```

Measured after the change: 5800. No clear change (-0.3%).
